# mprib/caliscope

Measured on AMD Instinct MI355X. Metric: observations/sec per LM iteration, higher is better.
Workload: dtype f64; 1 GPU; cfg4: 64 cams / 2000000 obs in total (200000 points / 2000000 obs on rank 0), extrinsics-only BA, linear loss; n_obs_total=2000000, params_per_camera=6, tolerances=ftol=xtol=gtol=1e-8 (reference defaults), sums=FP64 atomics (default)

## Files before the change

### caliscope_amd/build.py

```python

from __future__ import annotations

import os
import shutil
import subprocess
import sys
from pathlib import Path

HERE = Path(__file__).resolve().parent
CSRC = HERE / "csrc"
OUT = HERE / "libcaliscope_ba.so"
SOURCES = [CSRC / "cba_lib.hip", CSRC / "cba_solve.cpp", CSRC / "pose_lib.hip", CSRC / "scale_lib.hip", CSRC / "coverage_lib.hip", CSRC / "vertical_lib.hip", CSRC / "report_lib.hip", CSRC / "trajectory_lib.hip", CSRC / "covariance_lib.hip", CSRC / "reliability_lib.hip"]
DEPENDS = [CSRC / "cba_kernels.h", CSRC / "schur_plan.h", CSRC / "chol_schedule.h", CSRC / "chol_factor.h", CSRC / "host_plan.h", CSRC / "wg_binding.h", CSRC / "ba_math.h", CSRC / "trf_math.h", CSRC / "pnp_math.h", CSRC / "epipolar_math.h", CSRC / "intrinsic_math.h", CSRC / "frame_select_math.h", CSRC / "scale_math.h", CSRC / "coverage_math.h", CSRC / "vertical_math.h", CSRC / "report_math.h", CSRC / "trajectory_math.h", CSRC / "trajectory_refine_math.h", CSRC / "trajectory_cov_math.h", CSRC / "trajectory_smooth_math.h", CSRC / "covariance_math.h", CSRC / "covariance_constraint_math.h", CSRC / "covariance_constraint_plan.h", CSRC / "covariance_pipeline.h", CSRC / "reliability_math.h", CSRC / "reliability_constraint_math.h", CSRC / "device_call.h",
           HERE.parent / "include" / "caliscope_ba.h", HERE.parent / "include" / "caliscope_pose.h", HERE.parent / "include" / "caliscope_coverage.h", HERE.parent / "include" / "caliscope_vertical.h", HERE.parent / "include" / "caliscope_report.h", HERE.parent / "include" / "caliscope_trajectory.h", HERE.parent / "include" / "caliscope" / "uncertainty.h", HERE.parent / "include" / "caliscope" / "uncertainty_constrained.h",HERE.parent / "include" / "caliscope" / "reliability.h", HERE.parent / "include" / "caliscope" / "reliability_constrained.h",HERE.parent / "include" / "caliscope" / "trajectory_refine.h", HERE.parent / "include" / "caliscope" / "trajectory_uncertainty.h", HERE.parent / "include" / "caliscope" / "trajectory_smoother.h"]
ARCH = "gfx950"


def hipcc_path() -> str:
    for cand in (os.environ.get("HIPCC"), shutil.which("hipcc"), "/opt/rocm/bin/hipcc"):
        if cand and Path(cand).exists():
            return cand
    raise RuntimeError("hipcc not found (expected /opt/rocm/bin/hipcc)")


def needs_build() -> bool:
    if not OUT.exists():
        return True
    t = OUT.stat().st_mtime
    return any(p.stat().st_mtime > t for p in SOURCES + DEPENDS)


def source_digest() -> str:
    import hashlib

    h = hashlib.sha256()
    for path in sorted(SOURCES + DEPENDS, key=lambda q: q.name):
        h.update(path.name.encode())
        h.update(path.read_bytes())
    return h.hexdigest()


def built_digest(path: Path = OUT) -> str | None:
    import re

    m = re.search(rb"CBA_SOURCE_DIGEST=([0-9a-f]{64})", path.read_bytes())
    return m.group(1).decode() if m else None


def build(force: bool = False, verbose: bool = True) -> Path:
    if not force and not needs_build() and built_digest() == source_digest():
        return OUT
    cmd = [
        hipcc_path(), f"--offload-arch={ARCH}", "-O3", "-std=c++17", "-shared", "-fPIC", "-munsafe-fp-atomics",
        "-Wall", "-Wno-unused-function", f'-DCBA_SOURCE_DIGEST="{source_digest()}"', *map(str, SOURCES), "-o", str(OUT), "-pthread", "-lrccl",
        "-lrocprofiler-sdk-roctx",
    ]
    if verbose:
        print("[caliscope_amd.build]", " ".join(cmd), flush=True)
    subprocess.run(cmd, check=True, cwd=str(CSRC))
    return OUT


if __name__ == "__main__":
    build(force="--force" in sys.argv)
    print(OUT)
```

### caliscope_amd/csrc/ba_math.h

```cpp
#pragma once
#include <cstddef>
#include <cmath>
#include <cstdint>

#if defined(__HIPCC__)
#define CBA_HD __host__ __device__ __forceinline__
#else
#define CBA_HD inline
#endif

namespace cba {

constexpr int MODEL_PINHOLE_BC5 = 0;
constexpr int MODEL_FISHEYE4 = 1;
constexpr int CAM_CONST_STRIDE = 12;
constexpr int MAX_NC = 9;
constexpr double EPS_F64 = 2.220446049250313e-16;

CBA_HD double inv_sqrt(double x) {
#if defined(__HIP_DEVICE_COMPILE__)
  double y = __builtin_amdgcn_rsq(x);
  y = y * (1.5 - 0.5 * x * y * y);
  y = y * (1.5 - 0.5 * x * y * y);
  return y;
#else
  return 1.0 / sqrt(x);
#endif
}

enum Loss : int { LOSS_LINEAR = 0, LOSS_HUBER = 1, LOSS_SOFT_L1 = 2, LOSS_CAUCHY = 3, LOSS_ARCTAN = 4 };

struct CamTab {
  double R[9];
  double t[3];
  double Jl[9];
  double fx, fy, cx, cy;
  double d[5];
  double fx0, fy0, inv_fx0;
  double model;
  double nparams;
  double pad[13];
};
static_assert(sizeof(CamTab) == 48 * sizeof(double), "CamTab must be 48 doubles");
static_assert(offsetof(CamTab, pad) == 35 * sizeof(double), "35 doubles + pad[0] are live (CAMTAB_LIVE = 36 in cba_kernels.h)");
constexpr int CAMTAB_DOUBLES = 48;

CBA_HD void cam_prepare(const double* x_cam, const double* cconst, int model, int nparams, CamTab* o, int param_off = 0) {
  const double rx = x_cam[0], ry = x_cam[1], rz = x_cam[2];
  const double th2 = rx * rx + ry * ry + rz * rz;
  const double th = sqrt(th2);
  double ca, sa, a, b;
  if (th < 1e-4) {
    const double th4 = th2 * th2;
    a = 0.5 - th2 / 24.0 + th4 / 720.0;
    b = 1.0 / 6.0 - th2 / 120.0 + th4 / 5040.0;
    ca = 1.0 - th2 * a;
    sa = th - th2 * th * b;
  } else {
    ca = cos(th);
    sa = sin(th);
    a = (1.0 - ca) / th2;
    b = (th - sa) / (th2 * th);
  }
  const double sinc = (th < 1e-4) ? (1.0 - th2 / 6.0 + th2 * th2 / 120.0) : sa / th;
  const double xx = rx * rx, yy = ry * ry, zz = rz * rz, xy = rx * ry, xz = rx * rz, yz = ry * rz;
  o->R[0] = 1.0 + a * (xx - th2);  o->R[1] = -sinc * rz + a * xy;    o->R[2] = sinc * ry + a * xz;
  o->R[3] = sinc * rz + a * xy;    o->R[4] = 1.0 + a * (yy - th2);   o->R[5] = -sinc * rx + a * yz;
  o->R[6] = -sinc * ry + a * xz;   o->R[7] = sinc * rx + a * yz;     o->R[8] = 1.0 + a * (zz - th2);
  o->Jl[0] = 1.0 + b * (xx - th2); o->Jl[1] = -a * rz + b * xy;      o->Jl[2] = a * ry + b * xz;
  o->Jl[3] = a * rz + b * xy;      o->Jl[4] = 1.0 + b * (yy - th2);  o->Jl[5] = -a * rx + b * yz;
  o->Jl[6] = -a * ry + b * xz;     o->Jl[7] = a * rx + b * yz;       o->Jl[8] = 1.0 + b * (zz - th2);
  (void)ca;
  o->t[0] = x_cam[3]; o->t[1] = x_cam[4]; o->t[2] = x_cam[5];
  const double fx0 = cconst[0], fy0 = cconst[1];
  o->fx0 = fx0; o->fy0 = fy0; o->inv_fx0 = 1.0 / fx0;
  o->cx = cconst[2]; o->cy = cconst[3];
  const bool free_intr = nparams == 9;
  o->fx = free_intr ? x_cam[6] * fx0 : fx0;
  o->fy = free_intr ? x_cam[6] * fy0 : fy0;
  o->d[0] = free_intr ? x_cam[7] : cconst[4];
  o->d[1] = free_intr ? x_cam[8] : cconst[5];
  for (int i = 2; i < 5; ++i) o->d[i] = cconst[4 + i];
  o->model = (double)model;
  o->nparams = (double)nparams;
  o->pad[0] = (double)param_off;
  for (int i = 1; i < 13; ++i) o->pad[i] = 0.0;
}

struct Lens {
  double xd, yd;
  double dxx, dxy, dyx, dyy;
  double xr2, yr2, xr4, yr4;
};

CBA_HD void lens_pinhole(const double* d, double x, double y, Lens* L) {
  const double k1 = d[0], k2 = d[1], p1 = d[2], p2 = d[3], k3 = d[4];
  const double r2 = x * x + y * y, r4 = r2 * r2;
  const double cd = 1.0 + r2 * (k1 + r2 * (k2 + r2 * k3));
  const double dcd2 = 2.0 * (k1 + r2 * (2.0 * k2 + r2 * (3.0 * k3)));
  const double x2 = x + x, y2 = y + y;
  const double a1 = x2 * y, a2 = r2 + x2 * x, a3 = r2 + y2 * y;
  L->xd = x * cd + p1 * a1 + p2 * a2;
  L->yd = y * cd + p1 * a3 + p2 * a1;
  L->dxx = cd + x * x * dcd2 + p1 * y2 + 3.0 * p2 * x2;
  L->dxy = x * y * dcd2 + p1 * x2 + p2 * y2;
  L->dyx = L->dxy;
  L->dyy = cd + y * y * dcd2 + 3.0 * p1 * y2 + p2 * x2;
  L->xr2 = x * r2; L->yr2 = y * r2; L->xr4 = x * r4; L->yr4 = y * r4;
}

CBA_HD void lens_fisheye(const double* d, double x, double y, Lens* L) {
  const double r2 = x * x + y * y;
  const double r = sqrt(r2);
  if (r > 1e-8) {
    const double th = atan(r), t2 = th * th;
    const double poly = 1.0 + t2 * (d[0] + t2 * (d[1] + t2 * (d[2] + t2 * d[3])));
    const double dpoly = 1.0 + t2 * (3.0 * d[0] + t2 * (5.0 * d[1] + t2 * (7.0 * d[2] + t2 * 9.0 * d[3])));
    const double thd = th * poly;
    const double inv_r = 1.0 / r;
    const double cd = thd * inv_r;
    const double dcd_dr = (dpoly / (1.0 + r2) * r - thd) * inv_r * inv_r;
    const double g = dcd_dr * inv_r;
    L->xd = x * cd; L->yd = y * cd;
    L->dxx = cd + x * x * g; L->dxy = x * y * g; L->dyx = L->dxy; L->dyy = cd + y * y * g;
  } else {
    L->xd = x; L->yd = y;
    L->dxx = 1.0; L->dxy = 0.0; L->dyx = 0.0; L->dyy = 1.0;
  }
  L->xr2 = L->yr2 = L->xr4 = L->yr4 = 0.0;
}

CBA_HD void project_residual(const CamTab& c, double X, double Y, double Z, double u, double v, double* e) {
  const double Xc = c.t[0] + c.R[0] * X + c.R[1] * Y + c.R[2] * Z;
  const double Yc = c.t[1] + c.R[3] * X + c.R[4] * Y + c.R[5] * Z;
  const double Zc = c.t[2] + c.R[6] * X + c.R[7] * Y + c.R[8] * Z;
  const double iz = 1.0 / Zc;
  const double x = Xc * iz, y = Yc * iz;
  Lens L;
  if (c.model != 0.0) lens_fisheye(c.d, x, y, &L); else lens_pinhole(c.d, x, y, &L);
  e[0] = ((c.cx - u) + c.fx * L.xd) * c.inv_fx0;
  e[1] = ((c.cy - v) + c.fy * L.yd) * c.inv_fx0;
}

CBA_HD void project_full(const CamTab& c, double X, double Y, double Z, double u, double v,
                         double* e, double (*A)[MAX_NC], double (*B)[3]) {
  const double Y0 = c.R[0] * X + c.R[1] * Y + c.R[2] * Z;
  const double Y1 = c.R[3] * X + c.R[4] * Y + c.R[5] * Z;
  const double Y2 = c.R[6] * X + c.R[7] * Y + c.R[8] * Z;
  const double Zc = Y2 + c.t[2];
  const double iz = 1.0 / Zc;
  const double x = (Y0 + c.t[0]) * iz, y = (Y1 + c.t[1]) * iz;
  Lens L;
  if (c.model != 0.0) lens_fisheye(c.d, x, y, &L); else lens_pinhole(c.d, x, y, &L);
  const double s = c.inv_fx0;
  e[0] = ((c.cx - u) + c.fx * L.xd) * s;
  e[1] = ((c.cy - v) + c.fy * L.yd) * s;
  const double fxs = c.fx * s, fys = c.fy * s;
  const double g00 = fxs * L.dxx * iz, g01 = fxs * L.dxy * iz;
  const double g10 = fys * L.dyx * iz, g11 = fys * L.dyy * iz;
  const double G[2][3] = {{g00, g01, -(g00 * x + g01 * y)}, {g10, g11, -(g10 * x + g11 * y)}};
  for (int r = 0; r < 2; ++r) {
    A[r][3] = G[r][0]; A[r][4] = G[r][1]; A[r][5] = G[r][2];
    B[r][0] = G[r][0] * c.R[0] + G[r][1] * c.R[3] + G[r][2] * c.R[6];
    B[r][1] = G[r][0] * c.R[1] + G[r][1] * c.R[4] + G[r][2] * c.R[7];
    B[r][2] = G[r][0] * c.R[2] + G[r][1] * c.R[5] + G[r][2] * c.R[8];
  }
  for (int j = 0; j < 3; ++j) {
    const double m0 = c.Jl[j], m1 = c.Jl[3 + j], m2 = c.Jl[6 + j];
    const double c0 = m1 * Y2 - m2 * Y1, c1 = m2 * Y0 - m0 * Y2, c2 = m0 * Y1 - m1 * Y0;
    A[0][j] = G[0][0] * c0 + G[0][1] * c1 + G[0][2] * c2;
    A[1][j] = G[1][0] * c0 + G[1][1] * c1 + G[1][2] * c2;
  }
  if (c.nparams == 9.0) {
    A[0][6] = c.fx0 * L.xd * s; A[1][6] = c.fy0 * L.yd * s;
    A[0][7] = fxs * L.xr2;      A[1][7] = fys * L.yr2;
    A[0][8] = fxs * L.xr4;      A[1][8] = fys * L.yr4;
  }
}

template <bool RES>
CBA_HD void project_factors_impl(const CamTab& c, double X, double Y, double Z, double u, double v,
                                 double* e, double (*G)[3], double* Yr, double (*Aint)[3], double (*B)[3], double* nrm = nullptr) {
  const double Y0 = c.R[0] * X + c.R[1] * Y + c.R[2] * Z;
  const double Y1 = c.R[3] * X + c.R[4] * Y + c.R[5] * Z;
  const double Y2 = c.R[6] * X + c.R[7] * Y + c.R[8] * Z;
  Yr[0] = Y0; Yr[1] = Y1; Yr[2] = Y2;
  const double Zc = Y2 + c.t[2];
  const double iz = 1.0 / Zc;
  const double x = (Y0 + c.t[0]) * iz, y = (Y1 + c.t[1]) * iz;
  if (nrm) { nrm[0] = x; nrm[1] = y; nrm[2] = iz; }
  Lens L;
  if (c.model != 0.0) lens_fisheye(c.d, x, y, &L); else lens_pinhole(c.d, x, y, &L);
  const double s = c.inv_fx0;
  if constexpr (RES) {
    e[0] = ((c.cx - u) + c.fx * L.xd) * s;
    e[1] = ((c.cy - v) + c.fy * L.yd) * s;
  }
  const double fxs = c.fx * s, fys = c.fy * s;
  const double g00 = fxs * L.dxx * iz, g01 = fxs * L.dxy * iz;
  const double g10 = fys * L.dyx * iz, g11 = fys * L.dyy * iz;
  G[0][0] = g00; G[0][1] = g01; G[0][2] = -(g00 * x + g01 * y);
  G[1][0] = g10; G[1][1] = g11; G[1][2] = -(g10 * x + g11 * y);
  for (int r = 0; r < 2; ++r) {
    B[r][0] = G[r][0] * c.R[0] + G[r][1] * c.R[3] + G[r][2] * c.R[6];
    B[r][1] = G[r][0] * c.R[1] + G[r][1] * c.R[4] + G[r][2] * c.R[7];
    B[r][2] = G[r][0] * c.R[2] + G[r][1] * c.R[5] + G[r][2] * c.R[8];
  }
  const bool free_intr = c.nparams == 9.0;
  Aint[0][0] = free_intr ? c.fx0 * L.xd * s : 0.0; Aint[1][0] = free_intr ? c.fy0 * L.yd * s : 0.0;
  Aint[0][1] = free_intr ? fxs * L.xr2 : 0.0;      Aint[1][1] = free_intr ? fys * L.yr2 : 0.0;
  Aint[0][2] = free_intr ? fxs * L.xr4 : 0.0;      Aint[1][2] = free_intr ? fys * L.yr4 : 0.0;
}
CBA_HD void project_factors(const CamTab& c, double X, double Y, double Z, double u, double v,
                            double* e, double (*G)[3], double* Yr, double (*Aint)[3], double (*B)[3], double* nrm = nullptr) {
  project_factors_impl<true>(c, X, Y, Z, u, v, e, G, Yr, Aint, B, nrm);
}
CBA_HD void project_factors(const CamTab& c, double X, double Y, double Z, double (*G)[3], double* Yr, double (*Aint)[3], double (*B)[3],
                            double* nrm = nullptr) {
  project_factors_impl<false>(c, X, Y, Z, 0.0, 0.0, nullptr, G, Yr, Aint, B, nrm);
}

constexpr int REC6_VALUES = 10;
CBA_HD void rec6_head(const double* Yr, const double* t, double* nrm) {
  const double Zc = Yr[2] + t[2];
  const double iz = 1.0 / Zc;
  nrm[0] = (Yr[0] + t[0]) * iz; nrm[1] = (Yr[1] + t[1]) * iz; nrm[2] = iz;
}
CBA_HD void rec6_pack(const double (*G)[3], const double* Yr, const double (*Z)[3], double iz, double* rec) {
  rec[0] = Yr[0]; rec[1] = Yr[1]; rec[2] = Yr[2]; rec[3] = iz;
  for (int r = 0; r < 2; ++r)
    for (int k = 0; k < 3; ++k) rec[4 + 3 * r + k] = G[0][r] * Z[0][k] + G[1][r] * Z[1][k];
}
CBA_HD void rec6_pack(const double (*G)[3], const double* Yr, const double* t, const double (*Z)[3], double* rec) {
  double nrm[3];
  rec6_head(Yr, t, nrm);
  rec6_pack(G, Yr, Z, nrm[2], rec);
}
CBA_HD void rec6_xy(const double* rec, const double* t, double* x, double* y) {
  *x = (rec[0] + t[0]) * rec[3];
  *y = (rec[1] + t[1]) * rec[3];
}
CBA_HD void rec6_expand(const double* rec, const double* t, double* full) {
  double x, y;
  rec6_xy(rec, t, &x, &y);
  full[0] = rec[0]; full[1] = rec[1]; full[2] = rec[2];
  for (int k = 0; k < 3; ++k) {
    full[3 + k] = rec[4 + k]; full[6 + k] = rec[7 + k];
    full[9 + k] = -(x * rec[4 + k] + y * rec[7 + k]);
  }
}

CBA_HD double robust_one(int loss, double f_scale, double r, double* row_scale, double* r_scaled) {
  if (loss == LOSS_LINEAR) { *row_scale = 1.0; *r_scaled = r; return r * r; }
  const double fs2 = f_scale * f_scale;
  const double z = (r * r) / fs2;
  double rho0, rho1, rho2;
  switch (loss) {
    case LOSS_HUBER:
      if (z <= 1.0) { rho0 = z; rho1 = 1.0; rho2 = 0.0; }
      else { const double sz = sqrt(z); rho0 = 2.0 * sz - 1.0; rho1 = 1.0 / sz; rho2 = -0.5 / (z * sz); }
      break;
    case LOSS_SOFT_L1: {
      const double t = 1.0 + z, st = sqrt(t);
      rho0 = 2.0 * (st - 1.0); rho1 = 1.0 / st; rho2 = -0.5 / (t * st);
    } break;
    case LOSS_CAUCHY: {
      const double t = 1.0 + z;
      rho0 = log1p(z); rho1 = 1.0 / t; rho2 = -1.0 / (t * t);
    } break;
    default: {
      const double t = 1.0 + z * z;
      rho0 = atan(z); rho1 = 1.0 / t; rho2 = -2.0 * z / (t * t);
    } break;
  }
  double js = rho1 + 2.0 * rho2 * z;
  if (js < EPS_F64) js = EPS_F64;
  js = sqrt(js);
  *row_scale = js;
  *r_scaled = r * rho1 / js;
  return rho0 * fs2;
}

CBA_HD double robust_cost_one(int loss, double f_scale, double r) {
  if (loss == LOSS_LINEAR) return r * r;
  const double fs2 = f_scale * f_scale;
// ... 145 lines not shown
```

### caliscope_amd/csrc/cba_kernels.h

```cpp
#pragma once
#include <hip/hip_runtime.h>

#include "ba_math.h"
#include "trf_math.h"
#include "wg_binding.h"
#include "chol_schedule.h"

namespace cba {

constexpr int BLOCK = 256;
constexpr int CHUNK = 256;
constexpr int WAVE = 64;

struct VecLayout {
  int ncp;
  int ncp_pad;
  int P;
  int Ppad;
  __host__ __device__ long total() const { return (long)ncp_pad + 3L * Ppad; }
};

__device__ __forceinline__ double wave_sum(double v) {
#pragma unroll
  for (int o = WAVE / 2; o > 0; o >>= 1) v += __shfl_down(v, o, WAVE);
  return v;
}
__device__ __forceinline__ double wave_max(double v) {
#pragma unroll
  for (int o = WAVE / 2; o > 0; o >>= 1) v = fmax(v, __shfl_down(v, o, WAVE));
  return v;
}
#ifdef CBA_PROFILING
constexpr int STAMP_SLOTS = 96, STAMP_BLOCKS = 1024, STAMP_WAVES = 16, STAMP_ROW = 1 + STAMP_WAVES;
__device__ long long* g_cba_stamps = nullptr;
struct StampScope {
  long long* row;
  __device__ __forceinline__ explicit StampScope(int slot) : row(nullptr) {
    long long* base = g_cba_stamps;
    const int b = (int)(blockIdx.y * gridDim.x + blockIdx.x);
    if (base && slot < STAMP_SLOTS && b < STAMP_BLOCKS) {
      row = base + ((long)slot * STAMP_BLOCKS + b) * STAMP_ROW;
      if (threadIdx.x == 0 && threadIdx.y == 0) row[0] = wall_clock64();
    }
  }
  __device__ __forceinline__ ~StampScope() {
    const int t = (int)(threadIdx.y * blockDim.x + threadIdx.x);
    if (row && (t & (WAVE - 1)) == 0 && t / WAVE < STAMP_WAVES) row[1 + t / WAVE] = wall_clock64();
  }
};
#define CBA_STAMP(slot) StampScope cba_stamp_scope_(slot)
#else
#define CBA_STAMP(slot) ((void)0)
#endif
enum StampId { ST_TPREP = 0, ST_PAIRS, ST_REG_REDUCE, ST_FINALIZE, ST_CHOL_APPLY, ST_BACKSUB, ST_STEP_CAM, ST_BUILD, ST_REDUCE_PUB, ST_SCALE_LIN, ST_JV,
               ST_SMALL_SOLVE, ST_CHOL_STEP  };

__device__ __forceinline__ double block_sum(double v, double* sh) {
  v = wave_sum(v);
  const int lane = threadIdx.x & (WAVE - 1), w = threadIdx.x / WAVE;
  __syncthreads();
  if (lane == 0) sh[w] = v;
  __syncthreads();
  double r = 0.0;
  if (threadIdx.x == 0)
    for (int i = 0; i < BLOCK / WAVE; ++i) r += sh[i];
  return r;
}
__device__ __forceinline__ double block_max(double v, double* sh) {
  v = wave_max(v);
  const int lane = threadIdx.x & (WAVE - 1), w = threadIdx.x / WAVE;
  __syncthreads();
  if (lane == 0) sh[w] = v;
  __syncthreads();
  double r = 0.0;
  if (threadIdx.x == 0)
    for (int i = 0; i < BLOCK / WAVE; ++i) r = fmax(r, sh[i]);
  return r;
}

__device__ __forceinline__ void lds_add(double* addr, double v) { unsafeAtomicAdd(addr, v); }

constexpr int CAMTAB_LIVE = 36;
constexpr int CAMTAB_LDS = CAMTAB_LIVE + 1;
struct ObsRec { double u, v; int cam, pt; };
__device__ __forceinline__ ObsRec load_obs(const double* __restrict__ obs_u, const double* __restrict__ obs_v,
                                           const int* __restrict__ obs_cam, const int* __restrict__ obs_pt, int i) {
  ObsRec r;
  r.u = obs_u[i]; r.v = obs_v[i]; r.cam = obs_cam[i]; r.pt = obs_pt[i];
  return r;
}

__device__ __forceinline__ void stage_camtab(double* sh_tab, const double* tab, int n_cams) {
  for (int i = threadIdx.x; i < n_cams * CAMTAB_LIVE; i += BLOCK)
    sh_tab[(i / CAMTAB_LIVE) * CAMTAB_LDS + (i % CAMTAB_LIVE)] = tab[(i / CAMTAB_LIVE) * CAMTAB_DOUBLES + (i % CAMTAB_LIVE)];
}
__device__ __forceinline__ const CamTab& cam_at(const double* sh_tab, int cam) {
  return *reinterpret_cast<const CamTab*>(sh_tab + cam * CAMTAB_LDS);
}
template <bool CAMG>
__device__ __forceinline__ const CamTab& cam_of(const double* sh_tab, const double* __restrict__ tab, int cam) {
  if constexpr (CAMG) return *reinterpret_cast<const CamTab*>(tab + (long)cam * CAMTAB_DOUBLES);
  else return cam_at(sh_tab, cam);
}

__global__ void k_cam_prep(const double* __restrict__ xvec, const double* __restrict__ cam_const,
                           const int* __restrict__ cam_model, const int* __restrict__ cam_np,
                           const int* __restrict__ cam_off, int n_cams, double* __restrict__ tab) {
  const int c = blockIdx.x * blockDim.x + threadIdx.x;
  if (c >= n_cams) return;
  double xc[MAX_NC];
  const int np = cam_np[c];
  for (int i = 0; i < MAX_NC; ++i) xc[i] = (i < np) ? xvec[cam_off[c] + i] : 0.0;
  CamTab t;
  cam_prepare(xc, cam_const + c * CAM_CONST_STRIDE, cam_model[c], np, &t, cam_off[c]);
  const double* src = reinterpret_cast<const double*>(&t);
  for (int i = 0; i < CAMTAB_DOUBLES; ++i) tab[c * CAMTAB_DOUBLES + i] = src[i];
}

__global__ void __launch_bounds__(BLOCK)
k_begin(const double* __restrict__ x0, double* __restrict__ x, double* __restrict__ x_new, double* __restrict__ sinv, double* __restrict__ cam_diag,
        int* __restrict__ flags, long total, int ncp_pad, const double* __restrict__ cam_const, const int* __restrict__ cam_model,
        const int* __restrict__ cam_np, const int* __restrict__ cam_off, int n_cams, double* __restrict__ tab) {
  const long t0 = (long)blockIdx.x * blockDim.x + threadIdx.x;
  for (long i = t0; i < total; i += (long)gridDim.x * blockDim.x) {
    const double v = x0[i];
    x[i] = v;
    if (x_new) x_new[i] = v;
    sinv[i] = 1.0;
    if (i < ncp_pad) cam_diag[i] = 0.0;
    if (i < 4) flags[i] = 0;
  }
  if (t0 < n_cams) {
    const int c = (int)t0;
    double xc[MAX_NC];
    const int np = cam_np[c];
    for (int i = 0; i < MAX_NC; ++i) xc[i] = (i < np) ? x0[cam_off[c] + i] : 0.0;
    CamTab t;
    cam_prepare(xc, cam_const + c * CAM_CONST_STRIDE, cam_model[c], np, &t, cam_off[c]);
    const double* src = reinterpret_cast<const double*>(&t);
    for (int i = 0; i < CAMTAB_DOUBLES; ++i) tab[c * CAMTAB_DOUBLES + i] = src[i];
  }
}

template <bool WRITE_R, bool CAMG = false>
__global__ void __launch_bounds__(BLOCK)
k_cost(const double* __restrict__ obs_u, const double* __restrict__ obs_v, const int* __restrict__ obs_cam,
       const int* __restrict__ obs_pt, long n_obs, const double* __restrict__ xvec, VecLayout lay,
       const double* __restrict__ tab, int n_cams, int loss, double f_scale, double* __restrict__ partial,
       int* __restrict__ flags, double* __restrict__ r_out, const int* __restrict__ order) {
  extern __shared__ __attribute__((aligned(16))) double sh[];
  double* sh_tab = sh;
  double* sh_red = sh + (CAMG ? 0 : n_cams * CAMTAB_LDS);
  if (!CAMG) stage_camtab(sh_tab, tab, n_cams);
  __syncthreads();
  const double* px = xvec + lay.ncp_pad;
  double acc = 0.0;
  bool bad = false;
  struct Rec { int cam, pt; double u, v; long o; };
  const long stride = (long)gridDim.x * BLOCK, last = n_obs - 1;
  auto load_rec = [&](long i) {
    Rec r; const long k = min(i, last);
    r.cam = obs_cam[k]; r.pt = obs_pt[k]; r.u = obs_u[k]; r.v = obs_v[k]; r.o = WRITE_R ? (long)order[k] : 0;
    return r;
  };
  long i = (long)blockIdx.x * BLOCK + threadIdx.x;
  Rec rc = load_rec(i), rn = load_rec(i + stride);
  double X = px[rc.pt], Y = px[lay.Ppad + rc.pt], Z = px[2 * lay.Ppad + rc.pt];
  for (; i < n_obs; i += stride) {
    asm volatile("s_waitcnt vmcnt(0)" ::: "memory");
    asm volatile("" : "+v"(rc.cam), "+v"(rc.pt), "+v"(rc.u), "+v"(rc.v), "+v"(rc.o));
    asm volatile("" : "+v"(rn.cam), "+v"(rn.pt), "+v"(rn.u), "+v"(rn.v), "+v"(rn.o));
    asm volatile("" : "+v"(X), "+v"(Y), "+v"(Z));
    const double Xn = px[rn.pt], Yn = px[lay.Ppad + rn.pt], Zn = px[2 * lay.Ppad + rn.pt];
    const Rec rnn = load_rec(i + 2 * stride);
    __builtin_amdgcn_sched_barrier(0);
    double e[2];
    project_residual(cam_of<CAMG>(sh_tab, tab, rc.cam), X, Y, Z, rc.u, rc.v, e);
    if (!(isfinite(e[0]) && isfinite(e[1]))) bad = true;
    acc += robust_cost_one(loss, f_scale, e[0]) + robust_cost_one(loss, f_scale, e[1]);
    if (WRITE_R) {
      r_out[2 * rc.o] = e[0];
      r_out[2 * rc.o + 1] = e[1];
    }
    rc = rn; rn = rnn; X = Xn; Y = Yn; Z = Zn;
  }
  asm volatile("s_waitcnt vmcnt(0)" ::: "memory");
  if (bad) flags[0] = 1;
  const double tot = block_sum(acc, sh_red);
  if (threadIdx.x == 0) partial[blockIdx.x] = tot;
}

constexpr int REDUCE_RY = 16;
__device__ __forceinline__ void reduce_rows_block(const double* __restrict__ partial, int nrow, int width, double* __restrict__ out,
                                                  double* __restrict__ grad_out, const int* __restrict__ cam_off, const int* __restrict__ cam_np,
                                                  int stride, int tri) {
  __shared__ double sh[REDUCE_RY][64];
  const int j = blockIdx.x * 64 + threadIdx.x;
  double acc[8] = {0.0, 0.0, 0.0, 0.0, 0.0, 0.0, 0.0, 0.0};
  if (j < width) {
    int b = threadIdx.y;
    for (; b + 7 * REDUCE_RY < nrow; b += 8 * REDUCE_RY) {
#pragma unroll
      for (int q = 0; q < 8; ++q) acc[q] += partial[(long)(b + q * REDUCE_RY) * width + j];
    }
    for (; b < nrow; b += REDUCE_RY) acc[0] += partial[(long)b * width + j];
  }
  sh[threadIdx.y][threadIdx.x] = ((acc[0] + acc[1]) + (acc[2] + acc[3])) + ((acc[4] + acc[5]) + (acc[6] + acc[7]));
  __syncthreads();
  if (threadIdx.y == 0 && j < width) {
    double tot = 0.0;
#pragma unroll
    for (int y = 0; y < REDUCE_RY; ++y) tot += sh[y][threadIdx.x];
    out[j] = tot;
    if (grad_out) {
      const int c = j / stride, r = j % stride - tri;
      if (r >= 0 && r < cam_np[c]) grad_out[cam_off[c] + r] = tot;
    }
  }
}
__global__ void __launch_bounds__(64 * REDUCE_RY)
k_reduce_rows(const double* __restrict__ partial, int nrow, int width, double* __restrict__ out,
              double* __restrict__ grad_out = nullptr, const int* __restrict__ cam_off = nullptr, const int* __restrict__ cam_np = nullptr,
              int stride = 1, int tri = 0) {
  reduce_rows_block(partial, nrow, width, out, grad_out, cam_off, cam_np, stride, tri);
}
struct PubArgs {
  double* scal; int n_scal; int* flags; double* host_scal; int* host_flags; unsigned long long seq;
  const double* part_a; int rows_a, slot_a; const double* part_b; int rows_b, slot_b;
  const double* cam_src[4]; double* cam_dst; int ncp;
  int* spec_word; double ftol, xtol, cost_x;
};
__device__ __forceinline__ int pub_solve_ends(const PubArgs& pub, double ta, double tb) {
  const double cost_new = 0.5 * ta;
  const double cost = isnan(pub.cost_x) ? 0.5 * pub.scal[8] : pub.cost_x;
  if (pub.scal[42] != 0.0 || (pub.flags[0] | pub.flags[1] | pub.flags[2] | pub.flags[3]) != 0 || !isfinite(cost_new) || !isfinite(cost)) return 0;
  const double actual = cost - cost_new;
  const double ratio = trf::reduction_ratio(actual, pub.scal[45]);
  return trf::termination(actual, cost, sqrt(tb), sqrt(pub.scal[2]), ratio, pub.ftol, pub.xtol) != trf::TERMINATION_NONE ? 1 : 0;
}
__device__ __forceinline__ void publish_packet(const PubArgs& pub) {
  __shared__ double sh_w[2][REDUCE_RY];
  const int t = threadIdx.y * 64 + threadIdx.x;
  const double own = (t < pub.n_scal) ? pub.scal[t] : 0.0;
  double a = 0.0, b = 0.0;
  for (int r = t; r < pub.rows_a; r += 64 * REDUCE_RY) a += pub.part_a[r];
  for (int r = t; r < pub.rows_b; r += 64 * REDUCE_RY) b += pub.part_b[r];
  a = wave_sum(a); b = wave_sum(b);
  if (threadIdx.x == 0) { sh_w[0][threadIdx.y] = a; sh_w[1][threadIdx.y] = b; }
  __syncthreads();
  __shared__ double sh_tot[3];
  if (t == 0) {
    double ta = 0.0, tb = 0.0;
    for (int i = 0; i < REDUCE_RY; ++i) { ta += sh_w[0][i]; tb += sh_w[1][i]; }
    pub.scal[pub.slot_a] = ta; pub.scal[pub.slot_b] = tb;
    sh_tot[0] = ta; sh_tot[1] = tb;
    int ends = 0;
    if (pub.spec_word) { ends = pub_solve_ends(pub, ta, tb); *pub.spec_word = ends; }
    sh_tot[2] = (double)ends;
  }
  __syncthreads();
  if (t < pub.n_scal) pub.host_scal[t] = (t == pub.slot_a) ? sh_tot[0] : (t == pub.slot_b) ? sh_tot[1] : (t == pub.n_scal - 1) ? sh_tot[2] : own;
  if (t < 4) { pub.host_flags[t] = pub.flags[t]; pub.flags[t] = 0; }
  if (pub.cam_dst)
    for (int e = t; e < 4 * pub.ncp; e += 64 * REDUCE_RY) pub.cam_dst[e] = pub.cam_src[e / pub.ncp][e % pub.ncp];
  __threadfence_system();
  __syncthreads();
  if (t == 0) reinterpret_cast<volatile unsigned long long*>(pub.host_scal)[63] = pub.seq;
}
__global__ void __launch_bounds__(64 * REDUCE_RY)
k_reduce_rows_pub(const double* __restrict__ partial, int nrow, int width, double* __restrict__ out, double* __restrict__ grad_out,
                  const int* __restrict__ cam_off, const int* __restrict__ cam_np, int stride, int tri, PubArgs pub) {
  CBA_STAMP(ST_REDUCE_PUB);
  if (blockIdx.x + 1 < gridDim.x) { reduce_rows_block(partial, nrow, width, out, grad_out, cam_off, cam_np, stride, tri); return; }
  publish_packet(pub);
}
__global__ void k_xpack(const double* __restrict__ scal, const int* __restrict__ flags, unsigned long long mask, int with_max,
                        int rank, int world, double* __restrict__ xbuf) {
  if (threadIdx.x != 0 || blockIdx.x != 0) return;
  int n = 0;
  for (int s2 = 0; s2 < 32; ++s2)
    if ((mask >> s2) & 1ull) xbuf[n++] = scal[s2];
  for (int k = 0; k < 4; ++k) xbuf[n++] = flags[k] ? 1.0 : 0.0;
  if (with_max)
    for (int r = 0; r < world; ++r) xbuf[n++] = (r == rank) ? scal[4] : 0.0;
}
__global__ void k_xunpack(const double* __restrict__ xbuf, unsigned long long mask, int with_max, int world,
                          double* __restrict__ scal, int* __restrict__ flags) {
  if (threadIdx.x != 0 || blockIdx.x != 0) return;
  int n = 0;
  for (int s2 = 0; s2 < 32; ++s2)
    if ((mask >> s2) & 1ull) scal[s2] = xbuf[n++];
  for (int k = 0; k < 4; ++k) flags[k] = xbuf[n++] > 0.5 ? 1 : 0;
  if (with_max) {
    double m = 0.0;
    for (int r = 0; r < world; ++r) m = fmax(m, xbuf[n++]);
    scal[4] = m;
  }
}

template <bool MAX>
__global__ void __launch_bounds__(BLOCK)
k_reduce_narrow(const double* __restrict__ partial, int nrow, int width, double* __restrict__ out) {
  __shared__ double sh_red[BLOCK / WAVE];
  for (int j = 0; j < width; ++j) {
    double s = 0.0;
    for (int b = threadIdx.x; b < nrow; b += BLOCK) {
      const double v = partial[(long)b * width + j];
      s = MAX ? fmax(s, v) : s + v;
    }
    const double r = MAX ? block_max(s, sh_red) : block_sum(s, sh_red);
    if (threadIdx.x == 0) out[j] = r;
  }
}

template <int NC>
__device__ __forceinline__ double obs_linearize(const CamTab& c_lds, double X, double Y, double Z, double u, double v,
                                                int loss, double f_scale, double* e, double (*A)[MAX_NC],
                                                double (*B)[3]) {
  const CamTab c = c_lds;
  __builtin_amdgcn_sched_barrier(0);
  project_full(c, X, Y, Z, u, v, e, A, B);
  double rho = 0.0;
#pragma unroll
  for (int r = 0; r < 2; ++r) {
    double rs, er;
    rho += robust_one(loss, f_scale, e[r], &rs, &er);
    e[r] = er;
    if (loss != LOSS_LINEAR) {
#pragma unroll
      for (int k = 0; k < NC; ++k) A[r][k] *= rs;
      B[r][0] *= rs; B[r][1] *= rs; B[r][2] *= rs;
    }
  }
  return rho;
}

__device__ __forceinline__ double obs_factors(const CamTab& c_lds, double X, double Y, double Z, double u, double v, int loss, double f_scale, double* e,
                                              double (*G)[3], double* Yr, double (*Aint)[3], double (*B)[3], double* nrm = nullptr) {
  CamTab c;
  {
    const double* src = reinterpret_cast<const double*>(&c_lds);
    double* dst = reinterpret_cast<double*>(&c);
#pragma unroll
    for (int i = 0; i < 12; ++i) dst[i] = src[i];
#pragma unroll
    for (int i = 21; i < 35; ++i) dst[i] = src[i];
  }
  __builtin_amdgcn_sched_barrier(0);
  project_factors(c, X, Y, Z, u, v, e, G, Yr, Aint, B, nrm);
  if (nrm) {
#pragma unroll
    for (int k = 0; k < 3; ++k) asm("" : "+v"(nrm[k]));
  }
  double rho = 0.0;
#pragma unroll
  for (int r = 0; r < 2; ++r) {
    double rs, er;
    rho += robust_one(loss, f_scale, e[r], &rs, &er);
    e[r] = er;
    if (loss != LOSS_LINEAR) {
#pragma unroll
      for (int k = 0; k < 3; ++k) { G[r][k] *= rs; B[r][k] *= rs; Aint[r][k] *= rs; }
    }
  }
  return rho;
}
__device__ __forceinline__ void obs_factors(const CamTab& c_lds, double X, double Y, double Z, double (*G)[3], double* Yr, double (*Aint)[3], double (*B)[3],
                                            double* nrm = nullptr) {
  CamTab c;
  {
    const double* src = reinterpret_cast<const double*>(&c_lds);
    double* dst = reinterpret_cast<double*>(&c);
#pragma unroll
    for (int i = 0; i < 12; ++i) dst[i] = src[i];
    dst[21] = src[21]; dst[22] = src[22];
#pragma unroll
    for (int i = 25; i < 35; ++i) dst[i] = src[i];
  }
  __builtin_amdgcn_sched_barrier(0);
  project_factors(c, X, Y, Z, G, Yr, Aint, B, nrm);
#pragma unroll
  for (int r = 0; r < 2; ++r) {
#pragma unroll
    for (int k = 0; k < 3; ++k) { asm("" : "+v"(G[r][k])); asm("" : "+v"(B[r][k])); asm("" : "+v"(Aint[r][k])); }
  }
#pragma unroll
  for (int k = 0; k < 3; ++k) asm("" : "+v"(Yr[k]));
  if (nrm) {
#pragma unroll
    for (int k = 0; k < 3; ++k) asm("" : "+v"(nrm[k]));
  }
}

template <int NC> struct UPack {
  static constexpr int TRI = NC * (NC + 1) / 2;
  static constexpr int STRIDE = TRI + NC;
  __host__ __device__ static constexpr int idx(int r, int c) { return r * NC - r * (r - 1) / 2 + (c - r); }
};

constexpr int DET_ROUND = 9;
constexpr int DET_LD = CHUNK + 1;
struct DetPlan {
  const unsigned char* perm;
  const unsigned short* cstart;
};
template <int M>
__device__ __forceinline__ void det_round(const double* val, double* sh_cv, const int* sh_perm, const int* sh_cs, int n_cams, double* acc) {
#pragma unroll
  for (int q = 0; q < DET_ROUND; ++q) sh_cv[q * DET_LD + threadIdx.x] = val[q];
  __syncthreads();
#pragma unroll
  for (int m = 0; m < M; ++m) {
    const int task = (int)threadIdx.x + BLOCK * m;
    if (task < n_cams * DET_ROUND) {
      const int c = task / DET_ROUND, q = task % DET_ROUND;
      double s = 0.0;
      for (int j = sh_cs[c]; j < sh_cs[c + 1]; ++j) s += sh_cv[q * DET_LD + sh_perm[j]];
      acc[m] += s;
    }
  }
  __syncthreads();
}

template <int NC>
__device__ __forceinline__ double cam_block_value(int v, const double (*A)[MAX_NC], const double* e, int np) {
  using UP = UPack<NC>;
  int idx = 0;
#pragma unroll
  for (int r = 0; r < NC; ++r)
#pragma unroll
    for (int c = r; c < NC; ++c, ++idx)
      if (idx == v) return (r < np && c < np) ? A[0][r] * A[0][c] + A[1][r] * A[1][c] : 0.0;
#pragma unroll
  for (int r = 0; r < NC; ++r)
    if (UP::TRI + r == v) return (r < np) ? A[0][r] * e[0] + A[1][r] * e[1] : 0.0;
  return 0.0;
}

template <int NC, int DETM = 0, bool CAMG = false>
__global__ void __launch_bounds__(BLOCK)
k_build(const double* __restrict__ obs_u, const double* __restrict__ obs_v, const int* __restrict__ obs_cam,
        const int* __restrict__ obs_pt, const int* __restrict__ pt_start, const int* __restrict__ chunk_start,
        const int* __restrict__ chunk_pts, int n_chunks, const double* __restrict__ xvec, VecLayout lay, const double* __restrict__ tab, int n_cams,
        int loss, double f_scale, double* __restrict__ Vblk, double* __restrict__ gvec,
        double* __restrict__ partialU, double* __restrict__ partial_cost, int* __restrict__ flags, const double* __restrict__ skip,
        DetPlan det = DetPlan{nullptr, nullptr}) {
  using UP = UPack<NC>;
  constexpr bool DET = DETM > 0;
  if (skip && *skip != 0.0) return;
  extern __shared__ __attribute__((aligned(16))) double sh[];
  double* sh_tab = sh;
  double* sh_U = sh_tab + (CAMG ? 0 : n_cams * CAMTAB_LDS);
  auto cam_of = [&](int cam) -> const CamTab& {
    return CAMG ? *reinterpret_cast<const CamTab*>(tab + (long)cam * CAMTAB_DOUBLES) : cam_at(sh_tab, cam);
  };
  double* sh_pt = sh_U + (DET ? DET_ROUND * DET_LD : n_cams * UP::STRIDE);
  double* sh_red = sh_pt + 9 * CHUNK;
  int* sh_perm = reinterpret_cast<int*>(sh_red + 8);
  int* sh_cs = sh_perm + CHUNK;
  constexpr int DROUNDS = (UP::STRIDE + DET_ROUND - 1) / DET_ROUND;
  constexpr int DM = DET ? DETM : 1;
  double dacc[DROUNDS][DM];
#pragma unroll
  for (int r = 0; r < DROUNDS; ++r)
#pragma unroll
    for (int m = 0; m < DM; ++m) dacc[r][m] = 0.0;
  if (!CAMG) stage_camtab(sh_tab, tab, n_cams);
  if (!DET)
    for (int i = threadIdx.x; i < n_cams * UP::STRIDE; i += BLOCK) sh_U[i] = 0.0;
  __syncthreads();
  const double* px = xvec + lay.ncp_pad;
  double* gp = gvec + lay.ncp_pad;
  double cost = 0.0;
  bool bad = false;
  const int last_obs = max(chunk_start[n_chunks] - 1, 0);
  int ch = blockIdx.x;
  int o0 = 0, o1 = 0;
  ObsRec cur = {0.0, 0.0, 0, 0};
  if (ch < n_chunks) {
    o0 = chunk_start[ch]; o1 = chunk_start[ch + 1];
    cur = load_obs(obs_u, obs_v, obs_cam, obs_pt, min(o0 + (int)threadIdx.x, last_obs));
  }
  while (ch < n_chunks) {
    const int nxt = ch + gridDim.x, nc = min(nxt, n_chunks - 1);
    const int no0 = chunk_start[nc], no1 = chunk_start[nc + 1];
    const ObsRec nx = load_obs(obs_u, obs_v, obs_cam, obs_pt, min(no0 + (int)threadIdx.x, last_obs));
    const int cp0 = chunk_pts[2 * ch], npts = chunk_pts[2 * ch + 1];
    const int pp = min(cp0 + (int)threadIdx.x, lay.P - 1);
    const int pa = pt_start[pp] - o0, pb = pt_start[pp + 1] - o0;
    const int i = o0 + threadIdx.x;
    double pv[9];
#pragma unroll
    for (int q = 0; q < 9; ++q) pv[q] = 0.0;
    double e[2] = {0.0, 0.0}, A[2][MAX_NC];
    int np_det = 0;
    if (DET) {
#pragma unroll
      for (int k = 0; k < MAX_NC; ++k) { A[0][k] = 0.0; A[1][k] = 0.0; }
      sh_perm[threadIdx.x] = det.perm[(long)ch * CHUNK + threadIdx.x];
      for (int q = threadIdx.x; q <= n_cams; q += BLOCK) sh_cs[q] = det.cstart[(long)ch * (n_cams + 1) + q];
    }
    if (i < o1) {
      const int cam = cur.cam, pt = cur.pt;
      double B[2][3];
      cost += obs_linearize<NC>(cam_of(cam), px[pt], px[lay.Ppad + pt], px[2 * lay.Ppad + pt], cur.u, cur.v, loss,
                                f_scale, e, A, B);
      if (!isfinite(e[0] + e[1])) bad = true;
      pv[0] = B[0][0] * B[0][0] + B[1][0] * B[1][0];
      pv[1] = B[0][0] * B[0][1] + B[1][0] * B[1][1];
      pv[2] = B[0][0] * B[0][2] + B[1][0] * B[1][2];
      pv[3] = B[0][1] * B[0][1] + B[1][1] * B[1][1];
      pv[4] = B[0][1] * B[0][2] + B[1][1] * B[1][2];
      pv[5] = B[0][2] * B[0][2] + B[1][2] * B[1][2];
      pv[6] = B[0][0] * e[0] + B[1][0] * e[1];
      pv[7] = B[0][1] * e[0] + B[1][1] * e[1];
      pv[8] = B[0][2] * e[0] + B[1][2] * e[1];
      const int np = (int)cam_of(cam).nparams;
      np_det = np;
      if (!DET) {
        double* Uc = sh_U + cam * UP::STRIDE;
#pragma unroll
        for (int r = 0; r < NC; ++r) {
          if (r < np) {
#pragma unroll
            for (int c = r; c < NC; ++c)
              if (c < np) lds_add(&Uc[UP::idx(r, c)], A[0][r] * A[0][c] + A[1][r] * A[1][c]);
            lds_add(&Uc[UP::TRI + r], A[0][r] * e[0] + A[1][r] * e[1]);
          }
        }
      }
    }
#pragma unroll
    for (int q = 0; q < 9; ++q) sh_pt[q * CHUNK + threadIdx.x] = pv[q];
    __syncthreads();
    auto reduce_point = [&](int p, int a, int b) {
      double acc[9];
#pragma unroll
      for (int q = 0; q < 9; ++q) acc[q] = 0.0;
      for (int j = a; j < b; ++j) {
#pragma unroll
        for (int q = 0; q < 9; ++q) acc[q] += sh_pt[q * CHUNK + j];
      }
#pragma unroll
      for (int q = 0; q < 6; ++q) Vblk[(long)q * lay.Ppad + p] = acc[q];
      gp[p] = acc[6];
      gp[lay.Ppad + p] = acc[7];
      gp[2 * lay.Ppad + p] = acc[8];
    };
    if (npts < 0 && threadIdx.x < 9) {
      double acc = 0.0;
      for (int j = 0; j < o1 - o0; ++j) acc += sh_pt[threadIdx.x * CHUNK + j];
      if (threadIdx.x < 6) unsafeAtomicAdd(&Vblk[(long)threadIdx.x * lay.Ppad + cp0], acc);
      else unsafeAtomicAdd(&gp[(long)(threadIdx.x - 6) * lay.Ppad + cp0], acc);
    }
    if ((int)threadIdx.x < npts && pb > pa) reduce_point(pp, pa, pb);
    for (int lp = threadIdx.x + BLOCK; lp < npts; lp += BLOCK) {
      const int p = cp0 + lp;
      const int a = pt_start[p] - o0, b = pt_start[p + 1] - o0;
      if (b > a) reduce_point(p, a, b);
    }
    __syncthreads();
    if (DET) {
#pragma unroll
      for (int rd = 0; rd < DROUNDS; ++rd) {
        double val[DET_ROUND];
#pragma unroll
        for (int q = 0; q < DET_ROUND; ++q) val[q] = cam_block_value<NC>(rd * DET_ROUND + q, A, e, np_det);
        det_round<DM>(val, sh_U, sh_perm, sh_cs, n_cams, dacc[rd]);
      }
    }
    cur = nx; o0 = no0; o1 = no1; ch = nxt;
  }
  double* dst = partialU + (long)blockIdx.x * n_cams * UP::STRIDE;
  if (DET) {
#pragma unroll
    for (int rd = 0; rd < DROUNDS; ++rd)
#pragma unroll
      for (int m = 0; m < DM; ++m) {
        const int task = (int)threadIdx.x + BLOCK * m;
        const int c = task / DET_ROUND, v = rd * DET_ROUND + task % DET_ROUND;
        if (task < n_cams * DET_ROUND && v < UP::STRIDE) dst[c * UP::STRIDE + v] = dacc[rd][m];
      }
  } else {
    for (int i = threadIdx.x; i < n_cams * UP::STRIDE; i += BLOCK) dst[i] = sh_U[i];
  }
  const double tot = block_sum(cost, sh_red);
  if (threadIdx.x == 0) partial_cost[blockIdx.x] = tot;
  if (bad) flags[0] = 1;
}

constexpr int CS_MAX_PTS = 512;
struct CsPlan {
  const double* u;
  const double* v;
  const int* cam;
  const int* ptl;
  const int* obs_start;
  const int* pt_first;
  const int* pt_count;
  int n_sc;
  int pmax;
};
struct TrialSrc {
  const double *x, *g, *sinv, *s;
  const double* ab;
  double* x_new;
  double* step_partial;
};
template <int NC, bool CAMG = false, bool UGLOB = false, bool TRIAL = false>
__global__ void __launch_bounds__(BLOCK)
k_build_cs(CsPlan cs, const double* __restrict__ xvec, VecLayout lay, const double* __restrict__ tab, int n_cams, int loss, double f_scale,
           double* __restrict__ Vblk, double* __restrict__ gvec, double* __restrict__ partialU, double* __restrict__ partial_cost,
           int* __restrict__ flags, const double* __restrict__ skip, TrialSrc trial = TrialSrc{}) {
  CBA_STAMP(ST_BUILD);
  using UP = UPack<NC>;
  static_assert(!UGLOB || CAMG, "a camera count beyond the LDS copy of the blocks is beyond the LDS copy of the table as well");
  if (skip && *skip != 0.0) return;
  extern __shared__ __attribute__((aligned(16))) double sh[];
  double* sh_tab = sh;
  double* sh_U = sh_tab + (CAMG ? 0 : n_cams * CAMTAB_LDS);
  const int PM = cs.pmax;
  double* sh_vg = sh_U + (UGLOB ? 0 : n_cams * UP::STRIDE);
  double* sh_x = sh_vg + 9 * PM;
  double* sh_red = sh_x + 3 * PM;
  if (!CAMG) stage_camtab(sh_tab, tab, n_cams);
  if (!UGLOB)
    for (int i = threadIdx.x; i < n_cams * UP::STRIDE; i += BLOCK) sh_U[i] = 0.0;
  const double* px = xvec + lay.ncp_pad;
  double* gp = gvec + lay.ncp_pad;
  double cost = 0.0, step_sq = 0.0;
  const double t_alpha = TRIAL ? trial.ab[0] : 0.0, t_beta = TRIAL ? trial.ab[1] : 0.0;
  bool bad = false;
  for (int s = blockIdx.x; s < cs.n_sc; s += gridDim.x) {
    const int o0 = cs.obs_start[s], o1 = cs.obs_start[s + 1], p0 = cs.pt_first[s], npts = cs.pt_count[s];
    __syncthreads();
    for (int i = threadIdx.x; i < 9 * PM; i += BLOCK) sh_vg[i] = 0.0;
    if (TRIAL) {
      for (int i = threadIdx.x; i < npts; i += BLOCK) {
#pragma unroll
        for (int k = 0; k < 3; ++k) {
          const long e = (long)lay.ncp_pad + (long)k * lay.Ppad + p0 + i;
          const double si = trial.sinv[e];
          const double st = t_alpha * trial.g[e] / (si * si) + t_beta * trial.s[e];
          const double xn = trial.x[e] + st;
          trial.x_new[e] = xn;
          sh_x[k * PM + i] = xn;
          step_sq = fma(st, st, step_sq);
        }
      }
    } else {
      for (int i = threadIdx.x; i < npts; i += BLOCK) {
        sh_x[i] = px[p0 + i]; sh_x[PM + i] = px[lay.Ppad + p0 + i]; sh_x[2 * PM + i] = px[2 * lay.Ppad + p0 + i];
      }
    }
    __syncthreads();
    const int R = (o1 - o0 + BLOCK - 1) / BLOCK;
    const int j0 = o0 + (int)threadIdx.x * R, j1 = min(j0 + R, o1);
    double acc[UP::STRIDE];
#pragma unroll
    for (int q = 0; q < UP::STRIDE; ++q) acc[q] = 0.0;
    int cur_cam = -1, cur_np = 0;
    auto flush = [&]() {
      if (cur_cam < 0) return;
      double* Uc = (UGLOB ? partialU : sh_U) + (long)cur_cam * UP::STRIDE;
#pragma unroll
      for (int r = 0; r < NC; ++r) {
        if (r < cur_np) {
#pragma unroll
          for (int c = r; c < NC; ++c)
            if (c < cur_np) { if (UGLOB) atomicAdd(&Uc[UP::idx(r, c)], acc[UP::idx(r, c)]); else lds_add(&Uc[UP::idx(r, c)], acc[UP::idx(r, c)]); }
          if (UGLOB) atomicAdd(&Uc[UP::TRI + r], acc[UP::TRI + r]); else lds_add(&Uc[UP::TRI + r], acc[UP::TRI + r]);
        }
      }
#pragma unroll
      for (int q = 0; q < UP::STRIDE; ++q) acc[q] = 0.0;
    };
    const int jl = max(o1 - 1, 0);
    int n_cam = cs.cam[min(j0, jl)], n_pl = cs.ptl[min(j0, jl)];
    double n_u = cs.u[min(j0, jl)], n_v = cs.v[min(j0, jl)];
    for (int j = j0; j < j1; ++j) {
      asm volatile("s_waitcnt vmcnt(0)" ::: "memory");
      asm volatile("" : "+v"(n_cam), "+v"(n_pl), "+v"(n_u), "+v"(n_v));
      const int cam = n_cam, pl = n_pl;
      const double u = n_u, v = n_v;
      n_cam = cs.cam[min(j + 1, jl)]; n_pl = cs.ptl[min(j + 1, jl)]; n_u = cs.u[min(j + 1, jl)]; n_v = cs.v[min(j + 1, jl)];
      __builtin_amdgcn_sched_barrier(0);
      if (cam != cur_cam) { flush(); cur_cam = cam; cur_np = (int)cam_of<CAMG>(sh_tab, tab, cam).nparams; }
      double e[2], A[2][MAX_NC], B[2][3];
      {
        double G[2][3], Yr[3], Aint[2][3];
        const CamTab& ctc = cam_of<CAMG>(sh_tab, tab, cam);
        cost += obs_factors(ctc, sh_x[pl], sh_x[PM + pl], sh_x[2 * PM + pl], u, v, loss, f_scale, e, G, Yr, Aint, B);
#pragma unroll
        for (int r = 0; r < 2; ++r) {
          const double p0 = Yr[1] * G[r][2] - Yr[2] * G[r][1], p1 = Yr[2] * G[r][0] - Yr[0] * G[r][2], p2 = Yr[0] * G[r][1] - Yr[1] * G[r][0];
          if constexpr (UGLOB) {
            A[r][0] = ctc.Jl[0] * p0 + ctc.Jl[3] * p1 + ctc.Jl[6] * p2;
            A[r][1] = ctc.Jl[1] * p0 + ctc.Jl[4] * p1 + ctc.Jl[7] * p2;
            A[r][2] = ctc.Jl[2] * p0 + ctc.Jl[5] * p1 + ctc.Jl[8] * p2;
          } else {
            A[r][0] = p0; A[r][1] = p1; A[r][2] = p2;
          }
          A[r][3] = G[r][0]; A[r][4] = G[r][1]; A[r][5] = G[r][2];
          A[r][6] = Aint[r][0]; A[r][7] = Aint[r][1]; A[r][8] = Aint[r][2];
        }
      }
      if (!isfinite(e[0] + e[1])) bad = true;
#pragma unroll
      for (int r = 0; r < NC; ++r) {
#pragma unroll
        for (int c = r; c < NC; ++c) acc[UP::idx(r, c)] = fma(A[1][r], A[1][c], fma(A[0][r], A[0][c], acc[UP::idx(r, c)]));
        acc[UP::TRI + r] = fma(A[1][r], e[1], fma(A[0][r], e[0], acc[UP::TRI + r]));
      }
      lds_add(&sh_vg[0 * PM + pl], B[0][0] * B[0][0] + B[1][0] * B[1][0]);
      lds_add(&sh_vg[1 * PM + pl], B[0][0] * B[0][1] + B[1][0] * B[1][1]);
      lds_add(&sh_vg[2 * PM + pl], B[0][0] * B[0][2] + B[1][0] * B[1][2]);
      lds_add(&sh_vg[3 * PM + pl], B[0][1] * B[0][1] + B[1][1] * B[1][1]);
      lds_add(&sh_vg[4 * PM + pl], B[0][1] * B[0][2] + B[1][1] * B[1][2]);
      lds_add(&sh_vg[5 * PM + pl], B[0][2] * B[0][2] + B[1][2] * B[1][2]);
      lds_add(&sh_vg[6 * PM + pl], B[0][0] * e[0] + B[1][0] * e[1]);
      lds_add(&sh_vg[7 * PM + pl], B[0][1] * e[0] + B[1][1] * e[1]);
      lds_add(&sh_vg[8 * PM + pl], B[0][2] * e[0] + B[1][2] * e[1]);
    }
    flush();
    __syncthreads();
    for (int i = threadIdx.x; i < npts; i += BLOCK) {
#pragma unroll
      for (int q = 0; q < 6; ++q) Vblk[(long)q * lay.Ppad + p0 + i] = sh_vg[q * PM + i];
      gp[p0 + i] = sh_vg[6 * PM + i];
      gp[lay.Ppad + p0 + i] = sh_vg[7 * PM + i];
      gp[2 * lay.Ppad + p0 + i] = sh_vg[8 * PM + i];
    }
  }
  __syncthreads();
  if (!UGLOB) {
    for (int c = threadIdx.x; c < n_cams; c += BLOCK) {
      const double* Jl = tab + (long)c * CAMTAB_DOUBLES + 12;
      double* Uc = sh_U + (long)c * UP::STRIDE;
      double M[3][3], T[3][3];
#pragma unroll
      for (int r = 0; r < 3; ++r)
#pragma unroll
        for (int q = 0; q < 3; ++q) M[r][q] = Uc[UP::idx(min(r, q), max(r, q))];
#pragma unroll
      for (int r = 0; r < 3; ++r)
#pragma unroll
        for (int q = 0; q < 3; ++q) T[r][q] = Jl[r] * M[0][q] + Jl[3 + r] * M[1][q] + Jl[6 + r] * M[2][q];
#pragma unroll
      for (int r = 0; r < 3; ++r)
#pragma unroll
        for (int q = r; q < 3; ++q) Uc[UP::idx(r, q)] = T[r][0] * Jl[q] + T[r][1] * Jl[3 + q] + T[r][2] * Jl[6 + q];
#pragma unroll
      for (int q = 3; q <= NC; ++q) {
        double* v0 = (q < NC) ? &Uc[UP::idx(0, q)] : &Uc[UP::TRI + 0];
        double* v1 = (q < NC) ? &Uc[UP::idx(1, q)] : &Uc[UP::TRI + 1];
        double* v2 = (q < NC) ? &Uc[UP::idx(2, q)] : &Uc[UP::TRI + 2];
        const double a0 = *v0, a1 = *v1, a2 = *v2;
        *v0 = Jl[0] * a0 + Jl[3] * a1 + Jl[6] * a2;
        *v1 = Jl[1] * a0 + Jl[4] * a1 + Jl[7] * a2;
        *v2 = Jl[2] * a0 + Jl[5] * a1 + Jl[8] * a2;
      }
    }
    __syncthreads();
    double* dst = partialU + (long)blockIdx.x * n_cams * UP::STRIDE;
    for (int i = threadIdx.x; i < n_cams * UP::STRIDE; i += BLOCK) dst[i] = sh_U[i];
  }
  const double tot = block_sum(cost, sh_red);
  if (threadIdx.x == 0) partial_cost[blockIdx.x] = tot;
  if (TRIAL) {
    const double st = block_sum(step_sq, sh_red);
    if (threadIdx.x == 0) trial.step_partial[blockIdx.x] = st;
  }
  if (bad) flags[0] = 1;
}

__global__ void __launch_bounds__(256)
k_gather_uv(const double* __restrict__ uv_raw, const int* __restrict__ order, long n, double* __restrict__ u, double* __restrict__ v) {
  for (long i = (long)blockIdx.x * 256 + threadIdx.x; i < n; i += (long)gridDim.x * 256) {
    const double2 w = reinterpret_cast<const double2*>(uv_raw)[order[i]];
    u[i] = w.x; v[i] = w.y;
  }
}
__global__ void __launch_bounds__(256)
k_cs_fill(const int* __restrict__ perm, const int* __restrict__ sc_obs, const int* __restrict__ sc_p0, const double* __restrict__ u,
          const double* __restrict__ v, const int* __restrict__ cam, const int* __restrict__ pt, double* __restrict__ cu, double* __restrict__ cv,
          int* __restrict__ ccam, int* __restrict__ cptl) {
  const int s = blockIdx.x, o0 = sc_obs[s], o1 = sc_obs[s + 1], p0 = sc_p0[s];
  for (int j = o0 + threadIdx.x; j < o1; j += 256) {
    const int i = perm[j];
    cu[j] = u[i]; cv[j] = v[i]; ccam[j] = cam[i]; cptl[j] = pt[i] - p0;
  }
}

template <int NC>
__global__ void k_unpack_camera_grad(const double* __restrict__ Upacked, const int* __restrict__ cam_off,
                                     const int* __restrict__ cam_np, int n_cams, double* __restrict__ gvec) {
  using UP = UPack<NC>;
  const int t = blockIdx.x * blockDim.x + threadIdx.x;
  const int c = t / NC, r = t % NC;
  if (c >= n_cams || r >= cam_np[c]) return;
  gvec[cam_off[c] + r] = Upacked[c * UP::STRIDE + UP::TRI + r];
}

template <int NC>
__global__ void k_scale_update(const double* __restrict__ Upacked, const double* __restrict__ Vblk,
                               const int* __restrict__ param_cam, const int* __restrict__ param_loc, VecLayout lay,
                               int first, double* __restrict__ sinv, const double* __restrict__ cdiag) {
  using UP = UPack<NC>;
  const long total = lay.total();
  for (long i = (long)blockIdx.x * blockDim.x + threadIdx.x; i < total; i += (long)gridDim.x * blockDim.x) {
    double v;
    if (i < lay.ncp_pad) {
      if (i >= lay.ncp) continue;
      const int r = param_loc[i];
      v = Upacked[param_cam[i] * UP::STRIDE + UP::idx(r, r)];
    } else {
      const long k = (i - lay.ncp_pad) / lay.Ppad, p = (i - lay.ncp_pad) % lay.Ppad;
      if (p >= lay.P) continue;
      const int q = (k == 0) ? 0 : (k == 1 ? 3 : 5);
      v = Vblk[(long)q * lay.Ppad + p];
      if (cdiag) v += cdiag[k * lay.Ppad + p];
    }
    v = sqrt(v);
    if (first) { if (v == 0.0) v = 1.0; }
    else v = fmax(v, sinv[i]);
    sinv[i] = v;
  }
}

__global__ void k_cam_rescale(const double* __restrict__ state, const double* __restrict__ mult, const double* __restrict__ diag_h,
                              int ncp, double* __restrict__ sinv, double* __restrict__ cam_diag) {
  const int i = blockIdx.x * blockDim.x + threadIdx.x;
  if (i >= ncp) return;
  const double si = state[i] * mult[i];
  sinv[i] = si;
  cam_diag[i] = diag_h[i] * si * si;
}

__global__ void __launch_bounds__(BLOCK)
k_lin_scalars(const double* __restrict__ x, const double* __restrict__ g, const double* __restrict__ sinv,
              long total, int cam_end, int count_cams, int max_from, double* __restrict__ v1, double* __restrict__ partial,
              double* __restrict__ partial_max) {
  __shared__ double sh_red[BLOCK / WAVE];
  double s0 = 0, s1 = 0, s2 = 0, m = 0;
  for (long i = (long)blockIdx.x * BLOCK + threadIdx.x; i < total; i += (long)gridDim.x * BLOCK) {
    const double gi = g[i], si = sinv[i], xi = x[i];
    const double gh = gi / si;
    v1[i] = gh / si;
    if (i >= max_from) m = fmax(m, fabs(gi));
    if (i < cam_end && !count_cams) continue;
    s0 += gh * gh;
    s1 += (xi * si) * (xi * si);
    s2 += xi * xi;
  }
  double r;
  r = block_sum(s0, sh_red); if (threadIdx.x == 0) partial[blockIdx.x * 4 + 0] = r;
  r = block_sum(s1, sh_red); if (threadIdx.x == 0) partial[blockIdx.x * 4 + 1] = r;
  r = block_sum(s2, sh_red); if (threadIdx.x == 0) partial[blockIdx.x * 4 + 2] = r;
  if (threadIdx.x == 0) partial[blockIdx.x * 4 + 3] = 0.0;
  r = block_max(m, sh_red); if (threadIdx.x == 0) partial_max[blockIdx.x] = r;
}

__global__ void k_combine(const double* __restrict__ g, const double* __restrict__ sinv, const double* __restrict__ s,
                          double a, double b, long total, const double* __restrict__ over, int n_over, double* __restrict__ out) {
  for (long i = (long)blockIdx.x * blockDim.x + threadIdx.x; i < total; i += (long)gridDim.x * blockDim.x) {
    const double si = sinv[i];
    out[i] = (i < n_over) ? over[i] : a * g[i] / (si * si) + b * s[i];
  }
}

constexpr int MAIL_GNORM = 60, MAIL_GNORM_SEQ = 61;
struct SpecSkip {
  const int* word;
  const double* max_rows;
  int n_rows;
  double* mail; unsigned long long seq;
};
__device__ __forceinline__ void publish_gnorm(const SpecSkip& sk) {
  __shared__ double sh_gn[BLOCK / WAVE];
  double m = 0.0;
  for (int b = threadIdx.x; b < sk.n_rows; b += BLOCK) m = fmax(m, sk.max_rows[b]);
  m = block_max(m, sh_gn);
  if (threadIdx.x == 0) {
    sk.mail[MAIL_GNORM] = m;
    __threadfence_system();
    reinterpret_cast<volatile unsigned long long*>(sk.mail)[MAIL_GNORM_SEQ] = sk.seq;
  }
}
__global__ void __launch_bounds__(BLOCK) k_gnorm_pub(SpecSkip sk) { publish_gnorm(sk); }

template <int NC, int NV, bool CAMG = false, bool LIN = false>
__global__ void __launch_bounds__(BLOCK)
k_jv(const double* __restrict__ obs_u, const double* __restrict__ obs_v, const int* __restrict__ obs_cam,
     const int* __restrict__ obs_pt, long n_obs, const double* __restrict__ xvec, VecLayout lay,
     const double* __restrict__ tab, const int* __restrict__ cam_off, int n_cams, int loss, double f_scale,
     const double* __restrict__ v1, const double* __restrict__ v2, double* __restrict__ partial, SpecSkip skip = SpecSkip{}) {
  CBA_STAMP(ST_JV);
  if (skip.word && *skip.word) {
    if (blockIdx.x == 0) publish_gnorm(skip);
    return;
  }
  extern __shared__ __attribute__((aligned(16))) double sh[];
  double* sh_tab = sh;
  double* sh_v = sh_tab + (CAMG ? 0 : n_cams * CAMTAB_LDS);
  double* sh_red = sh_v + NV * lay.ncp_pad;
  if (!CAMG) stage_camtab(sh_tab, tab, n_cams);
  for (int i = threadIdx.x; i < lay.ncp_pad; i += BLOCK) {
    sh_v[i] = v1[i];
    if (NV == 2) sh_v[lay.ncp_pad + i] = v2[i];
  }
  __syncthreads();
  for (int c = threadIdx.x; c < n_cams; c += BLOCK) {
    const double* row = tab + (long)c * CAMTAB_DOUBLES;
    const int off = (int)row[35];
#pragma unroll
    for (int q = 0; q < NV; ++q) {
      double* vq = sh_v + q * lay.ncp_pad + off;
      const double r0 = vq[0], r1 = vq[1], r2 = vq[2];
      vq[0] = row[12] * r0 + row[13] * r1 + row[14] * r2;
      vq[1] = row[15] * r0 + row[16] * r1 + row[17] * r2;
      vq[2] = row[18] * r0 + row[19] * r1 + row[20] * r2;
    }
  }
  __syncthreads();
  const double* px = xvec + lay.ncp_pad;
  const double* p1 = v1 + lay.ncp_pad;
  const double* p2 = (NV == 2) ? v2 + lay.ncp_pad : nullptr;
  double s11 = 0, s12 = 0, s22 = 0;
  struct Rec { int cam, pt; double u, v; };
  struct Gat { double X, Y, Z, a, b, c, d, e, f; };
  constexpr int LOADS = (LIN ? 2 : 4) + (NV == 2 ? 9 : 6);
  const long stride = (long)gridDim.x * BLOCK, last = n_obs - 1;
  auto load_rec = [&](long i) {
    Rec r; const long k = min(i, last); r.cam = obs_cam[k]; r.pt = obs_pt[k];
    if constexpr (LIN) { r.u = r.v = 0.0; } else { r.u = obs_u[k]; r.v = obs_v[k]; }
    return r;
  };
  auto load_gat = [&](int pt) {
    Gat g;
    g.X = px[pt]; g.Y = px[lay.Ppad + pt]; g.Z = px[2 * lay.Ppad + pt];
    g.a = p1[pt]; g.b = p1[lay.Ppad + pt]; g.c = p1[2 * lay.Ppad + pt];
    if (NV == 2) { g.d = p2[pt]; g.e = p2[lay.Ppad + pt]; g.f = p2[2 * lay.Ppad + pt]; } else { g.d = g.e = g.f = 0.0; }
    return g;
  };
  auto launder_rec = [](Rec& r) {
    asm volatile("" : "+v"(r.cam), "+v"(r.pt));
    if constexpr (!LIN) asm volatile("" : "+v"(r.u), "+v"(r.v));
  };
  auto launder_gat = [](Gat& g) {
    asm volatile("" : "+v"(g.X), "+v"(g.Y), "+v"(g.Z), "+v"(g.a), "+v"(g.b), "+v"(g.c));
    if (NV == 2) asm volatile("" : "+v"(g.d), "+v"(g.e), "+v"(g.f));
  };
  long i = (long)blockIdx.x * BLOCK + threadIdx.x;
  Rec rc = load_rec(i), r1 = load_rec(i + stride), r2 = load_rec(i + 2 * stride), r3 = load_rec(i + 3 * stride);
  Gat gc = load_gat(rc.pt), g1 = load_gat(r1.pt);
  asm volatile("s_waitcnt vmcnt(0)" ::: "memory");
  launder_rec(rc); launder_rec(r1); launder_rec(r2); launder_rec(r3); launder_gat(gc); launder_gat(g1);
  for (; i < n_obs; i += stride) {
    asm volatile("s_waitcnt vmcnt(%0)" ::"n"(LOADS) : "memory");
    launder_gat(gc); launder_rec(r2);
    const Gat g2 = load_gat(r2.pt);
    const Rec r4 = load_rec(i + 4 * stride);
    __builtin_amdgcn_sched_barrier(0);
    const int cam = rc.cam;
    double e[2], G[2][3], Yr[3], Aint[2][3], B[2][3];
    const CamTab& ctj = cam_of<CAMG>(sh_tab, tab, cam);
    if constexpr (LIN) obs_factors(ctj, gc.X, gc.Y, gc.Z, G, Yr, Aint, B);
    else obs_factors(ctj, gc.X, gc.Y, gc.Z, rc.u, rc.v, loss, f_scale, e, G, Yr, Aint, B);
    const double* vc = sh_v + (int)ctj.pad[0];
    auto jv = [&](const double* q, double px0, double px1, double px2, double* o0, double* o1) {
      const double m0 = fma(q[1], Yr[2], fma(-q[2], Yr[1], q[3]));
      const double m1 = fma(q[2], Yr[0], fma(-q[0], Yr[2], q[4]));
      const double m2 = fma(q[0], Yr[1], fma(-q[1], Yr[0], q[5]));
      double a0 = B[0][0] * px0 + B[0][1] * px1 + B[0][2] * px2, a1 = B[1][0] * px0 + B[1][1] * px1 + B[1][2] * px2;
      a0 = fma(G[0][2], m2, fma(G[0][1], m1, fma(G[0][0], m0, a0)));
      a1 = fma(G[1][2], m2, fma(G[1][1], m1, fma(G[1][0], m0, a1)));
      if (NC == 9 && ctj.nparams == 9.0) {
        a0 = fma(Aint[0][2], q[8], fma(Aint[0][1], q[7], fma(Aint[0][0], q[6], a0)));
        a1 = fma(Aint[1][2], q[8], fma(Aint[1][1], q[7], fma(Aint[1][0], q[6], a1)));
      }
      *o0 = a0; *o1 = a1;
    };
    double a0, a1;
    jv(vc, gc.a, gc.b, gc.c, &a0, &a1);
    s11 += a0 * a0 + a1 * a1;
    if (NV == 2) {
      double b0, b1;
      jv(vc + lay.ncp_pad, gc.d, gc.e, gc.f, &b0, &b1);
      s12 += a0 * b0 + a1 * b1;
      s22 += b0 * b0 + b1 * b1;
    }
    rc = r1; r1 = r2; r2 = r3; r3 = r4; gc = g1; g1 = g2;
  }
  asm volatile("s_waitcnt vmcnt(0)" ::: "memory");
  double r;
  r = block_sum(s11, sh_red); if (threadIdx.x == 0) partial[blockIdx.x * 4 + 0] = r;
  r = block_sum(s12, sh_red); if (threadIdx.x == 0) partial[blockIdx.x * 4 + 1] = r;
  r = block_sum(s22, sh_red); if (threadIdx.x == 0) partial[blockIdx.x * 4 + 2] = r;
  if (threadIdx.x == 0) partial[blockIdx.x * 4 + 3] = 0.0;
}

struct TilePlan {
  const int* chunk_start;
  const int* wg_first;
  const int* wg_end;
  const int* wg_tile;
  const int* wg_stride;
  const int* tile_a;
  const int* tile_b;
  const int* group_cam_begin;
  const int* group_par_begin;
  int g;
  int tile_elems;
  const int* obs;
  int rep;
  const unsigned* codes;
  const int* code_start;
  const unsigned* nit;
  int prio_shift;
};

template <int NC> struct SchurRec {
  static constexpr int NVAL = (NC == 9) ? 21 : 10;
  static constexpr int NPH = (NVAL + 1) / 2;
  static constexpr int LST = (NPH & 1) ? NPH : NPH + 1;
  static constexpr int REC = 2 * LST;
  static constexpr int HREC = 2 * NPH;
  static constexpr int STAGE = (HREC / 2) | 1;
  static constexpr int STAGE_WAVES = (NC == 9) ? 2 : 4;
};
static_assert(SchurRec<6>::REC == 10 && SchurRec<6>::LST == 5 && SchurRec<6>::HREC == 10 && SchurRec<6>::STAGE == 5 && SchurRec<9>::REC == 22 &&
                  SchurRec<9>::LST == 11,
              "record sizes");

template <int NC>
__device__ __forceinline__ void expand_record(const double* __restrict__ rec, const double* __restrict__ cam_row, double* __restrict__ T) {
  const double* Jl = cam_row + 12;
  double full[12];
  if constexpr (NC == 6) rec6_expand(rec, cam_row + 9 , full);
  const double Y0 = (NC == 6) ? full[0] : rec[0], Y1 = (NC == 6) ? full[1] : rec[1], Y2 = (NC == 6) ? full[2] : rec[2];
  const double* Q = (NC == 6) ? full + 3 : rec + 3;
#pragma unroll
  for (int m = 0; m < 3; ++m) {
    const double q0 = Q[m], q1 = Q[3 + m], q2 = Q[6 + m];
    const double c0 = Y1 * q2 - Y2 * q1, c1 = Y2 * q0 - Y0 * q2, c2 = Y0 * q1 - Y1 * q0;
#pragma unroll
    for (int r = 0; r < 3; ++r) T[3 * r + m] = Jl[r] * c0 + Jl[3 + r] * c1 + Jl[6 + r] * c2;
    T[9 + m] = q0; T[12 + m] = q1; T[15 + m] = q2;
  }
  if (NC == 9) {
#pragma unroll
    for (int k = 0; k < 9; ++k) T[18 + k] = rec[12 + k];
  }
}

struct LinFin {
  const double* partial_lin;
  const double* partial_max;
  const double* partial_jv;
  int rows_lin, rows_jv;
  double radius;
  double* scal;
  double* fz;
};
__device__ __forceinline__ double lin_finish_block(const LinFin& lf, double (*sh_red)[BLOCK / WAVE], double* sh_out) {
  double v[10];
#pragma unroll
  for (int q = 0; q < 10; ++q) v[q] = 0.0;
  for (int b = threadIdx.x; b < lf.rows_lin; b += BLOCK) {
#pragma unroll
    for (int j = 0; j < 4; ++j) v[j] += lf.partial_lin[(long)b * 4 + j];
    v[4] = fmax(v[4], lf.partial_max[b]);
  }
  for (int b = threadIdx.x; b < lf.rows_jv; b += BLOCK) {
#pragma unroll
    for (int j = 0; j < 4; ++j) v[5 + j] += lf.partial_jv[(long)b * 4 + j];
  }
  const int lane = threadIdx.x & (WAVE - 1), w = threadIdx.x / WAVE;
#pragma unroll
  for (int q = 0; q < 9; ++q) {
    const double r = (q == 4) ? wave_max(v[q]) : wave_sum(v[q]);
    if (lane == 0) sh_red[q][w] = r;
  }
  __syncthreads();
  if (threadIdx.x == 0) {
    double tot[9];
#pragma unroll
    for (int q = 0; q < 9; ++q) {
      double r = 0.0;
      for (int i = 0; i < BLOCK / WAVE; ++i) r = (q == 4) ? fmax(r, sh_red[q][i]) : r + sh_red[q][i];
      tot[q] = r;
    }
    const double gh_sq = tot[0], jg_sq = tot[5] + tot[3], xs = sqrt(tot[1]);
    const double radius = lf.radius > 0.0 ? lf.radius : (xs > 0.0 ? xs : 1.0);
    const double lam = trf::damping(jg_sq, gh_sq, radius);
    sh_out[0] = lam;
    if (blockIdx.x == 0) {
#pragma unroll
      for (int q = 0; q < 9; ++q) lf.scal[q < 5 ? q : 12 + (q - 5)] = tot[q];
      lf.fz[0] = lam; lf.fz[1] = radius;
      lf.scal[40] = lam; lf.scal[41] = radius;
    }
  }
  __syncthreads();
  return sh_out[0];
}

template <int NC, int DETM = 0, bool CAMG = false, bool LINF = false, bool LIN = false>
__global__ void __launch_bounds__(BLOCK, DETM == 0 ? 2 : 1)
k_tprep(const double* __restrict__ obs_u, const double* __restrict__ obs_v, const int* __restrict__ obs_cam,
        const int* __restrict__ obs_pt, const int* __restrict__ chunk_start, int n_chunks,
        const double* __restrict__ xvec, VecLayout lay, const double* __restrict__ tab, const int* __restrict__ cam_off,
        int n_cams, int loss, double f_scale, double lam, const double* __restrict__ lam_dev, const double* __restrict__ Vblk,
        const double* __restrict__ gvec, const double* __restrict__ sinv, double* __restrict__ Trec,
        double* __restrict__ partial_b, int* __restrict__ flags, DetPlan det = DetPlan{nullptr, nullptr}, LinFin lf = LinFin{}) {
  CBA_STAMP(ST_TPREP);
  constexpr int REC = SchurRec<NC>::HREC, NP = REC / 2, SP = SchurRec<NC>::STAGE, SW = SchurRec<NC>::STAGE_WAVES;
  static_assert((BLOCK / WAVE) % SW == 0, "stage turns");
  constexpr bool DET = DETM > 0;
  static_assert(!(DET && CAMG), "the fixed-order sums keep the camera table in LDS");
  if (LINF) {
    __shared__ double sh_lf_red[10][BLOCK / WAVE];
    __shared__ double sh_lf_out[2];
    lam = lin_finish_block(lf, sh_lf_red, sh_lf_out);
  } else if (lam_dev) lam = *lam_dev;
  extern __shared__ __attribute__((aligned(16))) double sh[];
  double2* sh_stage = reinterpret_cast<double2*>(sh);
  double* sh_tab = sh + (size_t)SW * WAVE * SP * 2;
  double* sh_b = sh_tab + (CAMG ? 0 : n_cams * CAMTAB_LDS);
  int* sh_perm = reinterpret_cast<int*>(sh_b + DET_ROUND * DET_LD);
  int* sh_cs = sh_perm + CHUNK;
  constexpr int DM = DET ? DETM : 1;
  double dacc[DM];
#pragma unroll
  for (int m = 0; m < DM; ++m) dacc[m] = 0.0;
  stage_camtab(sh_tab, tab, n_cams);
  if (!DET)
    for (int i = threadIdx.x; i < lay.ncp_pad; i += BLOCK) sh_b[i] = 0.0;
  __syncthreads();
  const double* px = xvec + lay.ncp_pad;
  const double* gp = gvec + lay.ncp_pad;
  const double* dp = sinv + lay.ncp_pad;
  const int wv = threadIdx.x / WAVE, lane = threadIdx.x % WAVE;
  double2* stage = sh_stage + (wv % SW) * WAVE * SP;
  bool fail = false;
  const int last_obs = max(chunk_start[n_chunks] - 1, 0);
  constexpr bool PIPE = DETM == 0, FULL = true;
  struct PtOps { double X, Y, Z, V[6], d[3], g[3]; };
  auto load_rest = [&](PtOps& q, int pt) {
#pragma unroll
    for (int k = 0; k < 6; ++k) q.V[k] = Vblk[(long)k * lay.Ppad + pt];
#pragma unroll
    for (int k = 0; k < 3; ++k) { q.d[k] = dp[(long)k * lay.Ppad + pt]; q.g[k] = gp[(long)k * lay.Ppad + pt]; }
  };
  auto load_xyz = [&](PtOps& q, int pt) { q.X = px[pt]; q.Y = px[lay.Ppad + pt]; q.Z = px[2 * lay.Ppad + pt]; };
  auto load_ops = [&](int pt) {
    PtOps q;
    load_xyz(q, pt);
    if constexpr (FULL) load_rest(q, pt);
    return q;
  };
  auto load_rec = [&](int i) {
    if constexpr (LIN) return ObsRec{0.0, 0.0, obs_cam[i], obs_pt[i]};
    else return load_obs(obs_u, obs_v, obs_cam, obs_pt, i);
  };
  auto launder_obs = [](ObsRec& r) {
    if constexpr (!LIN) asm volatile("" : "+v"(r.u), "+v"(r.v));
    asm volatile("" : "+v"(r.cam), "+v"(r.pt));
  };
  auto launder_ops = [](PtOps& q) {
    asm volatile("" : "+v"(q.X), "+v"(q.Y), "+v"(q.Z));
    if constexpr (FULL) {
#pragma unroll
      for (int k = 0; k < 6; ++k) asm volatile("" : "+v"(q.V[k]));
#pragma unroll
      for (int k = 0; k < 3; ++k) asm volatile("" : "+v"(q.d[k]), "+v"(q.g[k]));
    }
  };
  const int stride = (int)gridDim.x, last_chunk = n_chunks - 1;
  int ch = blockIdx.x;
  int o0 = 0, o1 = 0, no0 = 0, no1 = 0;
  ObsRec cur = {0.0, 0.0, 0, 0}, nx = cur;
  PtOps ops;
  if (ch < n_chunks) {
    o0 = chunk_start[ch]; o1 = chunk_start[ch + 1];
    const int c1 = min(ch + stride, last_chunk);
    no0 = chunk_start[c1]; no1 = chunk_start[c1 + 1];
    cur = load_rec(min(o0 + (int)threadIdx.x, last_obs));
    if constexpr (PIPE) {
      if constexpr (FULL) nx = load_rec(min(no0 + (int)threadIdx.x, last_obs));
      else nx.pt = obs_pt[min(no0 + (int)threadIdx.x, last_obs)];
      ops = load_ops(cur.pt);
      asm volatile("s_waitcnt vmcnt(0)" ::: "memory");
      launder_obs(cur); launder_obs(nx); launder_ops(ops);
    }
  }
  while (ch < n_chunks) {
    const int nxt = ch + stride, c2 = min(ch + 2 * stride, last_chunk);
    const int nno0 = chunk_start[c2], nno1 = chunk_start[c2 + 1];
    PtOps ops_n;
    if constexpr (!PIPE) { load_xyz(ops, cur.pt); load_rest(ops, cur.pt); }
    else {
      if constexpr (!FULL) load_rest(ops, cur.pt);
      ops_n = load_ops(nx.pt);
    }
    ObsRec nn = {0.0, 0.0, 0, 0};
    if constexpr (PIPE && !FULL) {
      const int k1 = min(no0 + (int)threadIdx.x, last_obs);
      if constexpr (!LIN) { nx.u = obs_u[k1]; nx.v = obs_v[k1]; }
      nx.cam = obs_cam[k1];
      nn.pt = obs_pt[min(nno0 + (int)threadIdx.x, last_obs)];
    } else {
      nn = load_rec(min((PIPE ? nno0 : no0) + (int)threadIdx.x, last_obs));
    }
    if constexpr (PIPE) __builtin_amdgcn_sched_barrier(0);
    const int i = o0 + threadIdx.x;
    double rec[REC];
#pragma unroll
    for (int k = 0; k < REC; ++k) rec[k] = 0.0;
    double bval[DET_ROUND];
#pragma unroll
    for (int q = 0; q < DET_ROUND; ++q) bval[q] = 0.0;
    if (DET) {
      sh_perm[threadIdx.x] = det.perm[(long)ch * CHUNK + threadIdx.x];
      for (int q = threadIdx.x; q <= n_cams; q += BLOCK) sh_cs[q] = det.cstart[(long)ch * (n_cams + 1) + q];
    }
    if (i < o1) {
      const int cam = cur.cam;
      const CamTab& ct = cam_of<CAMG>(sh_tab, tab, cam);
      const double X = ops.X, Yw = ops.Y, Zw = ops.Z;
      double e[2], G[2][3], Yr[3], Aint[2][3], B[2][3], Z[2][3], nrm[3];
      if constexpr (LIN) obs_factors(ct, X, Yw, Zw, G, Yr, Aint, B, NC == 6 ? nrm : nullptr);
      else obs_factors(ct, X, Yw, Zw, cur.u, cur.v, loss, f_scale, e, G, Yr, Aint, B, NC == 6 ? nrm : nullptr);
      const int np = (int)ct.nparams;
      double Vd[6], L[6];
#pragma unroll
      for (int q = 0; q < 6; ++q) Vd[q] = ops.V[q];
      const double d0 = ops.d[0], d1 = ops.d[1], d2 = ops.d[2];
      Vd[0] += lam * d0 * d0; Vd[3] += lam * d1 * d1; Vd[5] += lam * d2 * d2;
      if (!chol3(Vd, L)) {
        fail = true;
        L[0] = L[2] = L[5] = 1.0; L[1] = L[3] = L[4] = 0.0;
      }
      chol3_fwd(L, B[0], Z[0]);
      chol3_fwd(L, B[1], Z[1]);
      const double gpt[3] = {ops.g[0], ops.g[1], ops.g[2]};
      double y[3];
      chol3_fwd(L, gpt, y);
      double* bc = sh_b + (int)ct.pad[0];
      rec[0] = Yr[0]; rec[1] = Yr[1]; rec[2] = Yr[2];
      double qy[3];
      if constexpr (NC == 6) {
        rec[3] = nrm[2];
#pragma unroll
        for (int r = 3; r < 5; ++r) {
          const double a0 = G[0][r - 3], a1 = G[1][r - 3];
          double t[3];
#pragma unroll
          for (int k = 0; k < 3; ++k) t[k] = a0 * Z[0][k] + a1 * Z[1][k];
          qy[r - 3] = t[0] * y[0] + t[1] * y[1] + t[2] * y[2];
          rec[3 * r - 5] = t[0]; rec[3 * r - 4] = t[1]; rec[3 * r - 3] = t[2];
        }
        qy[2] = -fma(nrm[0], qy[0], nrm[1] * qy[1]);
#pragma unroll
        for (int r = 3; r < 6; ++r) {
          if (DET) bval[r] = qy[r - 3];
          else lds_add(&bc[r], qy[r - 3]);
        }
      } else {
#pragma unroll
        for (int r = 3; r < NC; ++r) {
          const bool live = r < np;
          const double a0 = (r < 6) ? G[0][r - 3] : Aint[0][(r - 6) % 3], a1 = (r < 6) ? G[1][r - 3] : Aint[1][(r - 6) % 3];
          double t[3];
#pragma unroll
          for (int k = 0; k < 3; ++k) t[k] = live ? a0 * Z[0][k] + a1 * Z[1][k] : 0.0;
          const double ty = t[0] * y[0] + t[1] * y[1] + t[2] * y[2];
          if (r < 6) qy[r - 3] = ty;
          if (DET) bval[r] = live ? ty : 0.0;
          else if (live) lds_add(&bc[r], ty);
          rec[3 * r - 6] = t[0]; rec[3 * r - 5] = t[1]; rec[3 * r - 4] = t[2];
        }
      }
      {
        const double c0 = Yr[1] * qy[2] - Yr[2] * qy[1], c1 = Yr[2] * qy[0] - Yr[0] * qy[2], c2 = Yr[0] * qy[1] - Yr[1] * qy[0];
        if (DET) {
#pragma unroll
          for (int r = 0; r < 3; ++r) bval[r] = ct.Jl[r] * c0 + ct.Jl[3 + r] * c1 + ct.Jl[6 + r] * c2;
        } else {
          lds_add(&bc[0], c0); lds_add(&bc[1], c1); lds_add(&bc[2], c2);
        }
      }
    }
    if constexpr (PIPE) {
      asm volatile("s_waitcnt vmcnt(0)" ::: "memory");
      if constexpr (FULL) launder_obs(nn); else { launder_obs(nx); asm volatile("" : "+v"(nn.pt)); }
      launder_ops(ops_n);
    }
    const int w0 = o0 + wv * WAVE;
    const int n_pieces = max(0, min(WAVE, o1 - w0)) * NP;
    double2* dst = reinterpret_cast<double2*>(Trec + (long)w0 * REC);
#pragma unroll
    for (int turn = 0; turn < (BLOCK / WAVE) / SW; ++turn) {
      if (wv / SW == turn) {
#pragma unroll
        for (int k = 0; k < NP; ++k) stage[lane * SP + k] = make_double2(rec[2 * k], rec[2 * k + 1]);
        __builtin_amdgcn_fence(__ATOMIC_RELEASE, "wavefront");
        __builtin_amdgcn_wave_barrier();
        __builtin_amdgcn_fence(__ATOMIC_ACQUIRE, "wavefront");
#pragma unroll
        for (int k = 0; k < NP; ++k) {
          const int e = k * WAVE + lane;
          const double2 v = stage[(e / NP) * SP + e % NP];
          if (e < n_pieces) dst[e] = v;
        }
        __builtin_amdgcn_fence(__ATOMIC_RELEASE, "wavefront");
        __builtin_amdgcn_wave_barrier();
        __builtin_amdgcn_fence(__ATOMIC_ACQUIRE, "wavefront");
      }
      if (SW < BLOCK / WAVE) __syncthreads();
    }
    if (DET) {
      __syncthreads();
      det_round<DM>(bval, sh_b, sh_perm, sh_cs, n_cams, dacc);
    }
    if constexpr (PIPE && FULL) { cur = nx; nx = nn; ops = ops_n; }
    else if constexpr (PIPE) { cur = nx; nx.pt = nn.pt; ops.X = ops_n.X; ops.Y = ops_n.Y; ops.Z = ops_n.Z; }
    else { cur = nn; }
    o0 = no0; o1 = no1; no0 = nno0; no1 = nno1; ch = nxt;
  }
  if (fail) flags[1] = 1;
  __syncthreads();
  double* brow = partial_b + (long)blockIdx.x * lay.ncp_pad;
  if (DET) {
    for (int i = lay.ncp + threadIdx.x; i < lay.ncp_pad; i += BLOCK) brow[i] = 0.0;
#pragma unroll
    for (int m = 0; m < DM; ++m) {
      const int task = (int)threadIdx.x + BLOCK * m;
      const int c = task / DET_ROUND, q = task % DET_ROUND;
      if (task < n_cams * DET_ROUND && q < (int)cam_at(sh_tab, c).nparams) brow[cam_off[c] + q] = dacc[m];
    }
  } else {
    for (int c = threadIdx.x; c < n_cams; c += BLOCK) {
      const double* row = tab + (long)c * CAMTAB_DOUBLES;
      double* b3 = sh_b + (int)row[35];
      const double c0 = b3[0], c1 = b3[1], c2 = b3[2];
#pragma unroll
      for (int r = 0; r < 3; ++r) b3[r] = row[12 + r] * c0 + row[15 + r] * c1 + row[18 + r] * c2;
    }
    __syncthreads();
    for (int i = threadIdx.x; i < lay.ncp_pad; i += BLOCK) brow[i] = sh_b[i];
  }
}

__device__ __forceinline__ void pair9_corner(double (&acc)[6][6], const double2* __restrict__ Ri, const double2* __restrict__ Rj) {
  double D[3][3], Yi[3], Yj[3];
  {
    const double2 i0 = Ri[0], i1 = Ri[1], i2 = Ri[2], i3 = Ri[3], i4 = Ri[4], i5 = Ri[5];
    const double2 j0 = Rj[0], j1 = Rj[1], j2 = Rj[2], j3 = Rj[3], j4 = Rj[4], j5 = Rj[5];
    Yi[0] = i0.x; Yi[1] = i0.y; Yi[2] = i1.x; Yj[0] = j0.x; Yj[1] = j0.y; Yj[2] = j1.x;
    const double Qi[9] = {i1.y, i2.x, i2.y, i3.x, i3.y, i4.x, i4.y, i5.x, i5.y};
    const double Qj[9] = {j1.y, j2.x, j2.y, j3.x, j3.y, j4.x, j4.y, j5.x, j5.y};
#pragma unroll
    for (int a = 0; a < 3; ++a)
#pragma unroll
      for (int b = 0; b < 3; ++b) D[a][b] = fma(Qi[3 * a + 2], Qj[3 * b + 2], fma(Qi[3 * a + 1], Qj[3 * b + 1], Qi[3 * a] * Qj[3 * b]));
  }
  auto put = [&](int c, double m0, double m1, double m2) {
    acc[0][c] = fma(Yi[1], m2, fma(-Yi[2], m1, acc[0][c]));
    acc[1][c] = fma(Yi[2], m0, fma(-Yi[0], m2, acc[1][c]));
    acc[2][c] = fma(Yi[0], m1, fma(-Yi[1], m0, acc[2][c]));
    acc[3][c] += m0; acc[4][c] += m1; acc[5][c] += m2;
  };
#pragma unroll
  for (int b = 0; b < 3; ++b) put(3 + b, D[0][b], D[1][b], D[2][b]);
  put(0, fma(Yj[1], D[0][2], -(Yj[2] * D[0][1])), fma(Yj[1], D[1][2], -(Yj[2] * D[1][1])), fma(Yj[1], D[2][2], -(Yj[2] * D[2][1])));
  put(1, fma(Yj[2], D[0][0], -(Yj[0] * D[0][2])), fma(Yj[2], D[1][0], -(Yj[0] * D[1][2])), fma(Yj[2], D[2][0], -(Yj[0] * D[2][2])));
  put(2, fma(Yj[0], D[0][1], -(Yj[1] * D[0][0])), fma(Yj[0], D[1][1], -(Yj[1] * D[1][0])), fma(Yj[0], D[2][1], -(Yj[1] * D[2][0])));
}
__device__ __forceinline__ void pair9_cols(double* __restrict__ acc , const double2* __restrict__ Ri, const double2* __restrict__ Rj) {
  const double2 i0 = Ri[0], i1 = Ri[1], i2 = Ri[2], i3 = Ri[3], i4 = Ri[4], i5 = Ri[5], i6 = Ri[6], i7 = Ri[7], i8 = Ri[8], i9 = Ri[9], i10 = Ri[10];
  const double2 j6 = Rj[6], j7 = Rj[7], j8 = Rj[8], j9 = Rj[9], j10 = Rj[10];
  const double Yi[3] = {i0.x, i0.y, i1.x};
  const double Qi[9] = {i1.y, i2.x, i2.y, i3.x, i3.y, i4.x, i4.y, i5.x, i5.y};
  const double Ii[9] = {i6.x, i6.y, i7.x, i7.y, i8.x, i8.y, i9.x, i9.y, i10.x};
  const double Ij[9] = {j6.x, j6.y, j7.x, j7.y, j8.x, j8.y, j9.x, j9.y, j10.x};
#pragma unroll
  for (int b = 0; b < 3; ++b) {
    const double e0 = fma(Qi[2], Ij[3 * b + 2], fma(Qi[1], Ij[3 * b + 1], Qi[0] * Ij[3 * b]));
    const double e1 = fma(Qi[5], Ij[3 * b + 2], fma(Qi[4], Ij[3 * b + 1], Qi[3] * Ij[3 * b]));
    const double e2 = fma(Qi[8], Ij[3 * b + 2], fma(Qi[7], Ij[3 * b + 1], Qi[6] * Ij[3 * b]));
    acc[0 * 3 + b] = fma(Yi[1], e2, fma(-Yi[2], e1, acc[0 * 3 + b]));
    acc[1 * 3 + b] = fma(Yi[2], e0, fma(-Yi[0], e2, acc[1 * 3 + b]));
    acc[2 * 3 + b] = fma(Yi[0], e1, fma(-Yi[1], e0, acc[2 * 3 + b]));
    acc[3 * 3 + b] += e0; acc[4 * 3 + b] += e1; acc[5 * 3 + b] += e2;
#pragma unroll
    for (int a = 0; a < 3; ++a)
      acc[(6 + a) * 3 + b] = fma(Ii[3 * a + 2], Ij[3 * b + 2], fma(Ii[3 * a + 1], Ij[3 * b + 1], fma(Ii[3 * a], Ij[3 * b], acc[(6 + a) * 3 + b])));
  }
}
__device__ __forceinline__ void pair9_rows(double* __restrict__ acc , const double2* __restrict__ Ri, const double2* __restrict__ Rj) {
  const double2 i6 = Ri[6], i7 = Ri[7], i8 = Ri[8], i9 = Ri[9], i10 = Ri[10];
  const double2 j0 = Rj[0], j1 = Rj[1], j2 = Rj[2], j3 = Rj[3], j4 = Rj[4], j5 = Rj[5];
  const double Ii[9] = {i6.x, i6.y, i7.x, i7.y, i8.x, i8.y, i9.x, i9.y, i10.x};
  const double Yj[3] = {j0.x, j0.y, j1.x};
  const double Qj[9] = {j1.y, j2.x, j2.y, j3.x, j3.y, j4.x, j4.y, j5.x, j5.y};
#pragma unroll
  for (int a = 0; a < 3; ++a) {
    const double f0 = fma(Ii[3 * a + 2], Qj[2], fma(Ii[3 * a + 1], Qj[1], Ii[3 * a] * Qj[0]));
    const double f1 = fma(Ii[3 * a + 2], Qj[5], fma(Ii[3 * a + 1], Qj[4], Ii[3 * a] * Qj[3]));
    const double f2 = fma(Ii[3 * a + 2], Qj[8], fma(Ii[3 * a + 1], Qj[7], Ii[3 * a] * Qj[6]));
    acc[a * 6 + 3] += f0; acc[a * 6 + 4] += f1; acc[a * 6 + 5] += f2;
    acc[a * 6 + 0] = fma(Yj[1], f2, fma(-Yj[2], f1, acc[a * 6 + 0]));
    acc[a * 6 + 1] = fma(Yj[2], f0, fma(-Yj[0], f2, acc[a * 6 + 1]));
    acc[a * 6 + 2] = fma(Yj[0], f1, fma(-Yj[1], f0, acc[a * 6 + 2]));
  }
}

template <int NC> struct Reg3Cfg {
  static constexpr int REC = SchurRec<NC>::REC, LST = SchurRec<NC>::LST;
  static constexpr int SPLIT = (NC == 9) ? 3 : 1;
  static constexpr int CODE_THREADS = BLOCK, CODE_WAVES = BLOCK / WAVE;
  static constexpr int REG_BLOCK = BLOCK * SPLIT, NWAVES = REG_BLOCK / WAVE;
  static constexpr int GROUP = 16;
  static constexpr int NCD = (NC == 6) ? 8 : 4;
  static constexpr int PAIR_CAP = 0;
  static constexpr int SCHUNK = (NC == 9) ? 384 : 320;
  static constexpr int EPW = SCHUNK / NWAVES;
  static constexpr int NLD = (EPW * LST + WAVE - 1) / WAVE;
  static constexpr int WAVE_PIECES = NLD * WAVE;
  static constexpr int ZERO_PIECE = NWAVES * WAVE_PIECES;
  static constexpr int BUF_PIECES = ZERO_PIECE + LST + 1;
  static constexpr int NBUF = 2;
  static constexpr int SET_PIECES = NBUF * BUF_PIECES;
  static constexpr bool LANE_TABLE = (NC == 9);
  static constexpr int TABLE_PIECES = LANE_TABLE ? (NLD * WAVE * 4 + 15) / 16 : 0;
  static constexpr size_t LDS_BYTES = (size_t)(SET_PIECES + TABLE_PIECES) * 16;
  static constexpr int LAUNCH_THREADS = REG_BLOCK;
  static_assert(SCHUNK % NWAVES == 0 && EPW % 16 == 0 && EPW <= 2 * WAVE && (LST & 1) == 1, "staging layout");
  static_assert(ZERO_PIECE + LST < 65536, "piece addresses are 16 bit");
  static_assert(CODE_WAVES % 4 == 0, "iteration counts: four waves per word");
};

static_assert(Reg3Cfg<6>::EPW == 80 && Reg3Cfg<6>::LST == 5 && Reg3Cfg<6>::NLD == 7 && Reg3Cfg<6>::WAVE_PIECES == 448 && Reg3Cfg<6>::SCHUNK == 320 &&
                  Reg3Cfg<6>::ZERO_PIECE == 1792,
              "six-parameter pair kernel layout");

__device__ __forceinline__ void pair6(double (&acc)[6][6], const double2* __restrict__ Ri, const double2* __restrict__ Rj, double ti0, double ti1, double tj0,
                                      double tj1) {
  typedef double piece_t __attribute__((ext_vector_type(2)));
  const piece_t* Pi = reinterpret_cast<const piece_t*>(Ri);
  const piece_t* Pj = reinterpret_cast<const piece_t*>(Rj);
  const piece_t i0 = Pi[0], i1 = Pi[1], i2 = Pi[2], i3 = Pi[3], i4 = Pi[4];
  const piece_t j0 = Pj[0], j1 = Pj[1], j2 = Pj[2], j3 = Pj[3], j4 = Pj[4];
  const double Yi[3] = {i0.x, i0.y, i1.x}, Yj[3] = {j0.x, j0.y, j1.x};
  const double xi = (Yi[0] + ti0) * i1.y, yi = (Yi[1] + ti1) * i1.y, xj = (Yj[0] + tj0) * j1.y, yj = (Yj[1] + tj1) * j1.y;
  const double Qi[6] = {i2.x, i2.y, i3.x, i3.y, i4.x, i4.y};
  const double Qj[6] = {j2.x, j2.y, j3.x, j3.y, j4.x, j4.y};
  double M[3][6];
#pragma unroll
  for (int a = 0; a < 2; ++a) {
#pragma unroll
    for (int b2 = 0; b2 < 2; ++b2)
      M[a][3 + b2] = fma(Qi[3 * a + 2], Qj[3 * b2 + 2], fma(Qi[3 * a + 1], Qj[3 * b2 + 1], Qi[3 * a] * Qj[3 * b2]));
    M[a][5] = -fma(xj, M[a][3], yj * M[a][4]);
  }
#pragma unroll
  for (int b2 = 0; b2 < 3; ++b2) M[2][3 + b2] = -fma(xi, M[0][3 + b2], yi * M[1][3 + b2]);
#pragma unroll
  for (int a = 0; a < 3; ++a) {
    M[a][0] = fma(Yj[1], M[a][5], -(Yj[2] * M[a][4]));
    M[a][1] = fma(Yj[2], M[a][3], -(Yj[0] * M[a][5]));
    M[a][2] = fma(Yj[0], M[a][4], -(Yj[1] * M[a][3]));
  }
#pragma unroll
  for (int c = 0; c < 6; ++c) {
    acc[0][c] = fma(Yi[1], M[2][c], fma(-Yi[2], M[1][c], acc[0][c]));
    acc[1][c] = fma(Yi[2], M[0][c], fma(-Yi[0], M[2][c], acc[1][c]));
    acc[2][c] = fma(Yi[0], M[1][c], fma(-Yi[1], M[0][c], acc[2][c]));
    acc[3][c] += M[0][c]; acc[4][c] += M[1][c]; acc[5][c] += M[2][c];
  }
}

template <int NC, int RH>
__device__ __forceinline__ void unprime_rows(double (&acc)[RH][NC], int r0, const double* __restrict__ Ji, const double* __restrict__ Jj) {
  if (r0 == 0) {
#pragma unroll
    for (int c = 0; c < NC; ++c) {
      const double b0 = acc[0][c], b1 = acc[1][c], b2 = acc[2][c];
#pragma unroll
      for (int r = 0; r < 3; ++r) acc[r][c] = Ji[r] * b0 + Ji[3 + r] * b1 + Ji[6 + r] * b2;
    }
  }
#pragma unroll
  for (int r = 0; r < RH; ++r) {
    const double a0 = acc[r][0], a1 = acc[r][1], a2 = acc[r][2];
#pragma unroll
    for (int c = 0; c < 3; ++c) acc[r][c] = a0 * Jj[c] + a1 * Jj[3 + c] + a2 * Jj[6 + c];
  }
}

template <int NC, int SPLIT, bool CLK = false>
__device__ __forceinline__ void schur_reg3_body(const TilePlan& tp, const unsigned* __restrict__ p_nit, const int* __restrict__ p_code_start,
                                                const int* __restrict__ p_chunk_start, const unsigned* __restrict__ p_codes, const int* __restrict__ p_obs,
// ... 1128 lines not shown
  const int r = tid >> 4, cl = tid & 15, row = rj + r;
  double a0 = 0.0, a1 = 0.0;
  if (row < n) {
    const double* Tr = Tinv + (long)row * ldw;
    for (int c = rj + cl; c < k0; c += 32) { a0 = fma(Tr[c], Wn[c], a0); a1 = fma(Tr[c + 16], Wn[c + 16], a1); }
  }
  if constexpr (!EARLY) {
    chol_rank_nb(Wn + (k0 - NB), 1, W + (long)k0 * ldw + (k0 - NB), nbp, ldw, sh_red, wv, lane);
    __syncthreads();
  }
#pragma unroll
  for (int h = 0; h < EPT; ++h) {
    const int i = i0 + h * ISTEP;
    if constexpr (EARLY) sh_U[i][j] = m_ij[h];
    else sh_U[i][j] = m_ij[h] - sh_red[(i >> 4) * 2 + (j >> 4)][i & 15][j & 15];
    sh_L[i][j] = l_ij[h];
  }
  __syncthreads();
  if (wv < 2) {
    const int tj = wv;
    v4f64 c = {0.0, 0.0, 0.0, 0.0};
#pragma unroll
    for (int t = 0; t < NB / 4; ++t) {
      const int q = 4 * t + (lane >> 4);
      c = __builtin_amdgcn_mfma_f64_16x16x4f64(sh_U[lane & 15][q], sh_L[tj * 16 + (lane & 15)][q], c, 0, 0, 0);
    }
    if (lane < 16) sh_y[tj * 16 + lane] = (tj * 16 + lane < nbp) ? c[0] : 0.0;
  }
  __syncthreads();
  if (bj < k) {
    chol_rank_nb(Tinv + (long)rj * ldw + (k0 - NB), rcj, W + (long)k0 * ldw + (k0 - NB), nbp, ldw, sh_red, wv, lane);
    __syncthreads();
#pragma unroll
    for (int h = 0; h < EPT; ++h) {
      const int i = i0 + h * ISTEP;
      sh_U[i][j] = (i < rcj && j < nbp) ? old[h] + sh_red[(i >> 4) * 2 + (j >> 4)][i & 15][j & 15] : 0.0;
    }
    __syncthreads();
    if (wv < 4) {
      const int ti = wv >> 1, tj = wv & 1;
      v4f64 c = {0.0, 0.0, 0.0, 0.0};
#pragma unroll
      for (int t = 0; t < NB / 4; ++t) {
        const int q = 4 * t + (lane >> 4);
        c = __builtin_amdgcn_mfma_f64_16x16x4f64(sh_U[ti * 16 + (lane & 15)][q], sh_L[tj * 16 + (lane & 15)][q], c, 0, 0, 0);
      }
#pragma unroll
      for (int rr = 0; rr < 4; ++rr) sh_T[ti * 16 + (lane >> 4) + 4 * rr][tj * 16 + (lane & 15)] = -c[rr];
    }
  } else {
#pragma unroll
    for (int h = 0; h < EPT; ++h) sh_T[i0 + h * ISTEP][j] = old[h];
  }
  __syncthreads();
  if (row < n) {
    const int c = k0 + cl;
    if (c + 16 < n) { a0 = fma(sh_T[r][cl], sh_y[cl], a0); a1 = fma(sh_T[r][cl + 16], sh_y[cl + 16], a1); }
    else if (c < n) a0 = fma(sh_T[r][cl], sh_y[cl], a0);
  }
  double s = a0 + a1;
#pragma unroll
  for (int off = 8; off >= 1; off >>= 1) s += __shfl_xor(s, off, 16);
  if (cl == 0 && row < n) out[row] = s;
}

template <int NC, bool CAMG = false, bool SCAL = false>
__global__ void __launch_bounds__(BLOCK)
k_backsub(const double* __restrict__ obs_u, const double* __restrict__ obs_v, const int* __restrict__ obs_cam,
          const int* __restrict__ obs_pt, const int* __restrict__ pt_start, const int* __restrict__ chunk_start,
          const int* __restrict__ chunk_pts, int n_chunks, const double* __restrict__ xvec, VecLayout lay,
          const double* __restrict__ tab, const int* __restrict__ cam_off, int n_cams, int loss, double f_scale, double lam,
          const double* __restrict__ lam_dev, const double* __restrict__ Vblk, const double* __restrict__ gvec,
          const double* __restrict__ sinv, double* __restrict__ svec, double* __restrict__ step_partial = nullptr) {
  CBA_STAMP(ST_BACKSUB);
  extern __shared__ __attribute__((aligned(16))) double sh[];
  if (lam_dev) lam = *lam_dev;
  double* sh_tab = sh;
  double* sh_dc = sh_tab + (CAMG ? 0 : n_cams * CAMTAB_LDS);
  double* sh_pt = sh_dc + lay.ncp_pad;
  if (!CAMG) stage_camtab(sh_tab, tab, n_cams);
  for (int i = threadIdx.x; i < lay.ncp_pad; i += BLOCK) sh_dc[i] = svec[i];
  __syncthreads();
  for (int c = threadIdx.x; c < n_cams; c += BLOCK) {
    const double* row = tab + (long)c * CAMTAB_DOUBLES;
    double* d3 = sh_dc + (int)row[35];
    const double r0 = d3[0], r1 = d3[1], r2 = d3[2];
    d3[0] = row[12] * r0 + row[13] * r1 + row[14] * r2;
    d3[1] = row[15] * r0 + row[16] * r1 + row[17] * r2;
    d3[2] = row[18] * r0 + row[19] * r1 + row[20] * r2;
  }
  __syncthreads();
  const double* px = xvec + lay.ncp_pad;
  const double* gp = gvec + lay.ncp_pad;
  const double* dp = sinv + lay.ncp_pad;
  double* sp = svec + lay.ncp_pad;
  double sc0 = 0.0, sc1 = 0.0;
  auto solve_point = [&](int p, double* q, const double* Vin, const double* din, const double* gin) {
    double Vd[6], L[6], y[3], x[3];
#pragma unroll
    for (int k = 0; k < 6; ++k) Vd[k] = Vin[k];
    Vd[0] += lam * din[0] * din[0]; Vd[3] += lam * din[1] * din[1]; Vd[5] += lam * din[2] * din[2];
    if (chol3(Vd, L)) {
      chol3_fwd(L, q, y);
      chol3_bwd(L, y, x);
    } else {
      x[0] = x[1] = x[2] = 0.0;
    }
    sp[p] = -x[0];
    sp[lay.Ppad + p] = -x[1];
    sp[2 * lay.Ppad + p] = -x[2];
    if (SCAL) {
#pragma unroll
      for (int k = 0; k < 3; ++k) { const double ps = x[k] * din[k]; sc0 = fma(ps, ps, sc0); sc1 = fma(-gin[k], x[k], sc1); }
    }
  };
  const int last_obs = max(chunk_start[n_chunks] - 1, 0);
  int ch = blockIdx.x;
  int o0 = 0, o1 = 0;
  ObsRec cur = {0.0, 0.0, 0, 0};
  int pt_next = 0;
  double X = 0.0, Yw = 0.0, Zw = 0.0;
  if (ch < n_chunks) {
    o0 = chunk_start[ch]; o1 = chunk_start[ch + 1];
    cur = load_obs(obs_u, obs_v, obs_cam, obs_pt, min(o0 + (int)threadIdx.x, last_obs));
    pt_next = obs_pt[min(chunk_start[min(ch + (int)gridDim.x, n_chunks - 1)] + (int)threadIdx.x, last_obs)];
    X = px[cur.pt]; Yw = px[lay.Ppad + cur.pt]; Zw = px[2 * lay.Ppad + cur.pt];
  }
  while (ch < n_chunks) {
    const int nxt = ch + gridDim.x, nc = min(nxt, n_chunks - 1);
    const int no0 = chunk_start[nc], no1 = chunk_start[nc + 1];
    ObsRec nx;
    {
      const int k1 = min(no0 + (int)threadIdx.x, last_obs);
      nx.u = obs_u[k1]; nx.v = obs_v[k1]; nx.cam = obs_cam[k1]; nx.pt = pt_next;
    }
    const double Xn = px[pt_next], Yn = px[lay.Ppad + pt_next], Zn = px[2 * lay.Ppad + pt_next];
    const int pt_nn = obs_pt[min(chunk_start[min(nxt + (int)gridDim.x, n_chunks - 1)] + (int)threadIdx.x, last_obs)];
    const int cp0 = chunk_pts[2 * ch], npts = chunk_pts[2 * ch + 1];
    const int i = o0 + threadIdx.x;
    const int pp = min(cp0 + (int)threadIdx.x, lay.P - 1);
    int pa = 0, pb = 0;
    double Vp[6] = {0.0, 0.0, 0.0, 0.0, 0.0, 0.0}, dpp[3] = {0.0, 0.0, 0.0}, q[3] = {0.0, 0.0, 0.0}, gq[3] = {0.0, 0.0, 0.0};
    if (threadIdx.x < WAVE) {
      pa = pt_start[pp] - o0; pb = pt_start[pp + 1] - o0;
#pragma unroll
      for (int k = 0; k < 6; ++k) Vp[k] = Vblk[(long)k * lay.Ppad + pp];
#pragma unroll
      for (int k = 0; k < 3; ++k) { dpp[k] = dp[(long)k * lay.Ppad + pp]; q[k] = gp[(long)k * lay.Ppad + pp]; gq[k] = q[k]; }
    }
    double t[3] = {0.0, 0.0, 0.0};
    if (i < o1) {
      const int cam = cur.cam;
      double e[2], G[2][3], Yr[3], Aint[2][3], B[2][3];
      const CamTab& ctb = cam_of<CAMG>(sh_tab, tab, cam);
      obs_factors(ctb, X, Yw, Zw, cur.u, cur.v, loss, f_scale, e, G, Yr, Aint, B);
      const double* dc = sh_dc + (int)ctb.pad[0];
      const double m0 = fma(dc[1], Yr[2], fma(-dc[2], Yr[1], dc[3]));
      const double m1 = fma(dc[2], Yr[0], fma(-dc[0], Yr[2], dc[4]));
      const double m2 = fma(dc[0], Yr[1], fma(-dc[1], Yr[0], dc[5]));
      double a0 = fma(G[0][2], m2, fma(G[0][1], m1, G[0][0] * m0)), a1 = fma(G[1][2], m2, fma(G[1][1], m1, G[1][0] * m0));
      if (NC == 9 && ctb.nparams == 9.0) {
        a0 = fma(Aint[0][2], dc[8], fma(Aint[0][1], dc[7], fma(Aint[0][0], dc[6], a0)));
        a1 = fma(Aint[1][2], dc[8], fma(Aint[1][1], dc[7], fma(Aint[1][0], dc[6], a1)));
      }
      t[0] = B[0][0] * a0 + B[1][0] * a1;
      t[1] = B[0][1] * a0 + B[1][1] * a1;
      t[2] = B[0][2] * a0 + B[1][2] * a1;
    }
    sh_pt[threadIdx.x] = t[0];
    sh_pt[CHUNK + threadIdx.x] = t[1];
    sh_pt[2 * CHUNK + threadIdx.x] = t[2];
    __syncthreads();
    if (npts < 0 && threadIdx.x < 3) {
      double acc = 0.0;
      for (int j = 0; j < o1 - o0; ++j) acc += sh_pt[threadIdx.x * CHUNK + j];
      unsafeAtomicAdd(&sp[(long)threadIdx.x * lay.Ppad + cp0], acc);
    }
    if (threadIdx.x < WAVE && (int)threadIdx.x < npts && pb > pa) {
      for (int j = pa; j < pb; ++j) { q[0] += sh_pt[j]; q[1] += sh_pt[CHUNK + j]; q[2] += sh_pt[2 * CHUNK + j]; }
      solve_point(pp, q, Vp, dpp, gq);
    }
    for (int lp = (threadIdx.x < WAVE ? threadIdx.x + BLOCK : threadIdx.x); lp < npts; lp += BLOCK) {
      const int p = cp0 + lp;
      const int a = pt_start[p] - o0, b = pt_start[p + 1] - o0;
      if (b > a) {
        double q2[3] = {gp[p], gp[lay.Ppad + p], gp[2 * lay.Ppad + p]}, V2[6], d2[3];
        const double g2[3] = {q2[0], q2[1], q2[2]};
        for (int j = a; j < b; ++j) { q2[0] += sh_pt[j]; q2[1] += sh_pt[CHUNK + j]; q2[2] += sh_pt[2 * CHUNK + j]; }
#pragma unroll
        for (int k = 0; k < 6; ++k) V2[k] = Vblk[(long)k * lay.Ppad + p];
#pragma unroll
        for (int k = 0; k < 3; ++k) d2[k] = dp[(long)k * lay.Ppad + p];
        solve_point(p, q2, V2, d2, g2);
      }
    }
    __syncthreads();
    cur = nx; o0 = no0; o1 = no1; ch = nxt;
    pt_next = pt_nn; X = Xn; Yw = Yn; Zw = Zn;
  }
  if (SCAL) {
    double r;
    r = block_sum(sc0, sh_pt); if (threadIdx.x == 0) step_partial[blockIdx.x * 4 + 0] = r;
    r = block_sum(sc1, sh_pt); if (threadIdx.x == 0) { step_partial[blockIdx.x * 4 + 1] = r; step_partial[blockIdx.x * 4 + 2] = 0.0; step_partial[blockIdx.x * 4 + 3] = 0.0; }
  }
}

constexpr int BSR_PT = 3 * CHUNK;
template <int NC> struct BsrCfg {
  static constexpr int NP = SchurRec<NC>::NPH;
  static constexpr int CS = (NC == 9) ? 9 : 8;
  static constexpr int CSS = CS;
  static constexpr size_t lds_bytes(int n_cams) { return ((size_t)BLOCK * NP * 2 + 2 * BSR_PT + (size_t)n_cams * CSS + 8) * sizeof(double); }
};
template <int NC, bool SCAL>
__device__ __forceinline__ void backsub_rec_body(const double* __restrict__ Trec, const int* __restrict__ obs_cam, const int* __restrict__ pt_start,
                                                 const int* __restrict__ chunk_start, const int* __restrict__ chunk_pts, int n_chunks, VecLayout lay,
                                                 const double* __restrict__ tab, const int* __restrict__ cam_off, const int* __restrict__ cam_np,
                                                 int n_cams, double lam, const double* __restrict__ Vblk, const double* __restrict__ gp,
                                                 const double* __restrict__ dp, const double* __restrict__ s_cam, double* __restrict__ sp,
                                                 double* __restrict__ step_partial, double* sh) {
  using Cfg = BsrCfg<NC>;
  constexpr int NP = Cfg::NP, CSS = Cfg::CSS;
  double2* sh_rec = reinterpret_cast<double2*>(sh);
  double* sh_pt = sh + (size_t)BLOCK * NP * 2;
  double* sh_step = sh_pt + 2 * BSR_PT;
  const int tid = (int)threadIdx.x, lane = tid % WAVE;
  const int wv = __builtin_amdgcn_readfirstlane(tid / WAVE);
  for (int idx = tid; idx < n_cams * 3; idx += BLOCK) {
    const int c = idx / 3, a = idx % 3, off = cam_off[c];
    const double* Jl = tab + (long)c * CAMTAB_DOUBLES + 12;
    sh_step[c * CSS + a] = fma(Jl[3 * a + 2], s_cam[off + 2], fma(Jl[3 * a + 1], s_cam[off + 1], Jl[3 * a] * s_cam[off]));
    sh_step[c * CSS + 3 + a] = s_cam[off + 3 + a];
    if (NC == 9) sh_step[c * CSS + 6 + a] = (cam_np[c] == 9) ? s_cam[off + 6 + a] : 0.0;
    if (NC == 6 && a < 2) sh_step[c * CSS + 6 + a] = tab[(long)c * CAMTAB_DOUBLES + 9 + a];
  }
  const int n_obs = chunk_start[n_chunks];
  const int last_obs = max(n_obs - 1, 0);
  const long last_piece = (long)max(n_obs, 1) * NP - 1;
  const double2* rec_g = reinterpret_cast<const double2*>(Trec);
  double2* wrec = sh_rec + wv * (WAVE * NP);
  auto issue = [&](int o0) {
    const long base = ((long)o0 + wv * WAVE) * NP + lane;
#pragma unroll
    for (int k = 0; k < NP; ++k)
      __builtin_amdgcn_global_load_lds((const void __attribute__((address_space(1)))*)(rec_g + min(base + k * WAVE, last_piece)),
                                       (void __attribute__((address_space(3)))*)(wrec + k * WAVE), 16, 0, 0);
  };
  struct PtIn { int p, a, b, on; double V[6], d[3], g[3]; };
  const int lp0 = lane * 4 + wv;
  auto load_point = [&](int cp0, int npts) {
    PtIn q;
    q.on = lp0 < npts;
    q.p = min(cp0 + min(lp0, max(npts - 1, 0)), lay.P - 1);
    q.a = pt_start[q.p]; q.b = pt_start[q.p + 1];
#pragma unroll
    for (int k = 0; k < 6; ++k) q.V[k] = Vblk[(long)k * lay.Ppad + q.p];
#pragma unroll
    for (int k = 0; k < 3; ++k) { q.d[k] = dp[(long)k * lay.Ppad + q.p]; q.g[k] = gp[(long)k * lay.Ppad + q.p]; }
    return q;
  };
  double sc0 = 0.0, sc1 = 0.0;
  auto solve_point = [&](int p, const double* Vin, const double* din, const double* gin, const double* q) {
    double Vd[6], L[6], y[3], x[3];
#pragma unroll
    for (int k = 0; k < 6; ++k) Vd[k] = Vin[k];
    Vd[0] = fma(lam * din[0], din[0], Vd[0]); Vd[3] = fma(lam * din[1], din[1], Vd[3]); Vd[5] = fma(lam * din[2], din[2], Vd[5]);
    if (chol3(Vd, L)) {
      chol3_fwd(L, gin, y);
      y[0] += q[0]; y[1] += q[1]; y[2] += q[2];
      chol3_bwd(L, y, x);
    } else {
      x[0] = x[1] = x[2] = 0.0;
    }
    sp[p] = -x[0];
    sp[lay.Ppad + p] = -x[1];
    sp[2 * lay.Ppad + p] = -x[2];
    if (SCAL) {
#pragma unroll
      for (int k = 0; k < 3; ++k) { const double ps = x[k] * din[k]; sc0 = fma(ps, ps, sc0); sc1 = fma(-gin[k], x[k], sc1); }
    }
  };
  auto point_phase = [&](const PtIn& q, const double* pt, int cp0, int npts, int o0) {
    if (q.on && q.b > q.a) {
      double acc[3] = {0.0, 0.0, 0.0};
      for (int j = q.a - o0; j < q.b - o0; ++j) { acc[0] += pt[j]; acc[1] += pt[CHUNK + j]; acc[2] += pt[2 * CHUNK + j]; }
      solve_point(q.p, q.V, q.d, q.g, acc);
    }
    for (int lp = tid + BLOCK; lp < npts; lp += BLOCK) {
      const int p = cp0 + lp, a = pt_start[p] - o0, b = pt_start[p + 1] - o0;
      if (b > a) {
        double acc[3] = {0.0, 0.0, 0.0}, V2[6], d2[3], g2[3];
        for (int j = a; j < b; ++j) { acc[0] += pt[j]; acc[1] += pt[CHUNK + j]; acc[2] += pt[2 * CHUNK + j]; }
#pragma unroll
        for (int k = 0; k < 6; ++k) V2[k] = Vblk[(long)k * lay.Ppad + p];
#pragma unroll
        for (int k = 0; k < 3; ++k) { d2[k] = dp[(long)k * lay.Ppad + p]; g2[k] = gp[(long)k * lay.Ppad + p]; }
        solve_point(p, V2, d2, g2, acc);
      }
    }
  };

  int ch = blockIdx.x;
  if (ch >= n_chunks) {
    if (SCAL && tid == 0) { step_partial[blockIdx.x * 4 + 0] = 0.0; step_partial[blockIdx.x * 4 + 1] = 0.0; step_partial[blockIdx.x * 4 + 2] = 0.0; step_partial[blockIdx.x * 4 + 3] = 0.0; }
    return;
  }
  struct Ent { int o0, o1, cp0, npts; };
  auto load_ent = [&](int c) { Ent e; e.o0 = chunk_start[c]; e.o1 = chunk_start[c + 1]; e.cp0 = chunk_pts[2 * c]; e.npts = chunk_pts[2 * c + 1]; return e; };
  const int stride = (int)gridDim.x, last_chunk = n_chunks - 1;
// ... 1316 lines not shown
```

### caliscope_amd/csrc/cba_lib.hip

```cpp
#include <hip/hip_runtime.h>

#include <algorithm>
#include <atomic>
#include <chrono>
#include <cmath>
#include <condition_variable>
#include <cstdarg>
#include <cstdio>
#include <cstdlib>
#include <cstring>
#include <map>
#include <mutex>
#include <shared_mutex>
#include <memory>
#include <string>
#include <type_traits>
#include <thread>
#include <utility>
#include <vector>

#include <rccl/rccl.h>
#include <rocprofiler-sdk-roctx/roctx.h>

#include "../../include/caliscope_ba.h"
// ... 561 lines not shown
  std::sort(rows.begin(), rows.end(), [](const Row& a, const Row& b) { return a.t0 < b.t0; });
  size_t first = 0;
  for (size_t i = 0; i < rows.size(); ++i) if (rows[i].slot == ST_TPREP) first = i;
  fprintf(stderr, "device stamps of the last fused iteration (100 MHz wall clock; blocks = workgroups seen, at most %d):\n", STAMP_BLOCKS);
  fprintf(stderr, "| # | kernel | workgroups | first entry -> last exit, us | last entry after the first, us | workgroup lifetime min / mean / max, us | idle before, us |\n|---|---|---|---|---|---|---|\n");
  double busy = 0.0, idle = 0.0;
  for (size_t i = first; i < rows.size(); ++i) {
    const Row& r = rows[i];
    char nm[48];
    if (r.slot == ST_CHOL_STEP + 1 && chol_pairs(p)) snprintf(nm, sizeof nm, "k_chol_step k=-1 and 0");
    else if (r.slot >= ST_CHOL_STEP) snprintf(nm, sizeof nm, "k_chol_step k=%d", r.slot - ST_CHOL_STEP - 1); else snprintf(nm, sizeof nm, "%s", names[r.slot]);
    const double gap = i > first ? (r.t0 - rows[i - 1].t1) * 0.01 : 0.0;
    busy += (r.t1 - r.t0) * 0.01; if (i > first) idle += gap;
    fprintf(stderr, "| %zu | %s | %d | %.2f | %.2f | %.2f / %.2f / %.2f | %.2f |\n", i - first + 1, nm, r.blocks, (r.t1 - r.t0) * 0.01, (r.last_entry - r.t0) * 0.01,
            r.life_min * 0.01, r.life_sum / r.blocks * 0.01, r.life_max * 0.01, gap);
  }
  for (size_t i = 0; i < first; ++i) {
    const Row& r = rows[i];
    if (r.slot != ST_JV) continue;
    fprintf(stderr, "| (earlier) | %s | %d | %.2f | %.2f | %.2f / %.2f / %.2f | - |\n", names[r.slot], r.blocks, (r.t1 - r.t0) * 0.01,
            (r.last_entry - r.t0) * 0.01, r.life_min * 0.01, r.life_sum / r.blocks * 0.01, r.life_max * 0.01);
  }
  if (first < rows.size())
    fprintf(stderr, "%zu kernels, %.1f us inside kernels, %.1f us between them, %.1f us from the first entry to the last exit\n", rows.size() - first, busy, idle,
            (rows.back().t1 - rows[first].t0) * 0.01);
  if (!p->h_tile_wg_begin.empty() && p->tile_grid <= STAMP_BLOCKS) {
    const std::vector<int>& wgb = p->h_tile_wg_begin;
    const int nT = (int)wgb.size() - 1;
    std::vector<double> life(p->tile_grid, 0.0);
    for (int b = 0; b < p->tile_grid; ++b) {
      const long long* q = &h[((size_t)ST_PAIRS * STAMP_BLOCKS + b) * STAMP_ROW];
      long long e = 0;
      for (int w = 0; w < STAMP_WAVES; ++w) e = std::max(e, q[1 + w]);
      life[logical_workgroup(b, p->tile_grid)] = q[0] ? (e - q[0]) * 0.01 : 0.0;
    }
    fprintf(stderr, "k_schur_reg3 workgroup lifetimes by tile (us): tile: workgroups min / mean / max\n");
    for (int t = 0; t < nT; ++t) {
      double mn = 1e300, mx = 0.0, sm = 0.0;
      for (int b = wgb[t]; b < wgb[t + 1]; ++b) { mn = std::min(mn, life[b]); mx = std::max(mx, life[b]); sm += life[b]; }
      fprintf(stderr, "  %d: %d  %.1f / %.1f / %.1f\n", t, wgb[t + 1] - wgb[t], mn, sm / std::max(1, wgb[t + 1] - wgb[t]), mx);
    }
    fprintf(stderr, "... by XCD (logical id mod 8): min / mean / max\n");
    for (int x = 0; x < 8; ++x) {
      double mn = 1e300, mx = 0.0, sm = 0.0; int n = 0;
      for (int b = x; b < p->tile_grid; b += 8) { mn = std::min(mn, life[b]); mx = std::max(mx, life[b]); sm += life[b]; ++n; }
      fprintf(stderr, "  XCD %d: %.1f / %.1f / %.1f\n", x, mn, sm / std::max(1, n), mx);
    }
    fprintf(stderr, "... by dispatch order (hardware workgroup id, eighths of the grid): mean\n ");
    for (int o = 0; o < 8; ++o) {
      double sm = 0.0; int n = 0;
      for (int b = o * p->tile_grid / 8; b < (o + 1) * p->tile_grid / 8; ++b) { sm += life[logical_workgroup(b, p->tile_grid)]; ++n; }
      fprintf(stderr, " %.1f", sm / std::max(1, n));
    }
    fprintf(stderr, "\n");
  }
  (void)hipFree(p->stamps);
  p->stamps = nullptr;
}
#endif

void cba_destroy(cba_problem* p) {
  if (!p) return;
  drop_plan_task(p);
  (void)hipSetDevice(p->device);
  if (p->stream) (void)hipStreamSynchronize(p->stream);
  upload_stage_release(p);
#ifdef CBA_PROFILING
  if (p->stamps) dump_stamps(p);
#endif
  drain_timers(p);
  for (auto& ev : p->free_events) { (void)hipEventDestroy(ev.a); (void)hipEventDestroy(ev.b); }
  if (p->h_vec_sent) (void)hipEventDestroy(p->h_vec_sent);
  if (ncclComm_t c = p->comm.exchange(nullptr)) (void)ncclCommDestroy(c);
  {
    std::lock_guard<std::mutex> lock(g_pool_mu);
    DevicePool& pool = g_pool[p->device];
    for (size_t i = 0; i < p->allocs.size(); ++i) {
      if (p->alloc_bytes[i] == kPoolChunk && pool.chunks.size() < kPoolKeep) pool.chunks.push_back(p->allocs[i]);
      else (void)hipFree(p->allocs[i]);
    }
    if (p->h_scal) {
      if (pool.mail.size() < kPoolKeep) pool.mail.emplace_back(p->h_scal, p->mail_doubles);
      else (void)hipHostFree(p->h_scal);
    }
    if (p->h_vec) {
      if (pool.staging.size() < kPoolKeep && p->h_vec_doubles <= kPoolStagingMax) pool.staging.emplace_back(p->h_vec, p->h_vec_doubles);
      else (void)hipHostFree(p->h_vec);
    }
    if (p->stream) {
      if (pool.streams.size() < kPoolKeep) pool.streams.push_back(p->stream);
      else (void)hipStreamDestroy(p->stream);
    }
  }
  delete p;
}

}

static int raise_lds_ceiling(const void* fn, size_t bytes) {
  static std::mutex mu;
  static std::map<std::pair<int, const void*>, size_t> ceiling;
  int dev = 0;
  HIPCHK(hipGetDevice(&dev));
  std::lock_guard<std::mutex> lock(mu);
  size_t& have = ceiling[{dev, fn}];
  if (bytes <= have) return CBA_OK;
  HIPCHK(hipFuncSetAttribute(fn, hipFuncAttributeMaxDynamicSharedMemorySize, (int)bytes));
  have = bytes;
  return CBA_OK;
}

template <int NC> constexpr bool LIN_FORM = NC == 6;
template <int NC> static bool linear_pass_now(const cba_problem* p) { return LIN_FORM<NC> && p->linear_pass && p->loss == LOSS_LINEAR; }

template <typename K>
static int allow_lds(K kernel, size_t bytes) {
  if (bytes > 160 * 1024) return fail(CBA_ERR_UNSUPPORTED, "kernel needs %zu bytes of LDS (> 160 KiB)", bytes);
  return raise_lds_ceiling(reinterpret_cast<const void*>(kernel), bytes);
}

template <typename K>
static int resident_per_cu(K kernel, size_t lds, int fallback) {
  int n = 0;
  if (hipOccupancyMaxActiveBlocksPerMultiprocessor(&n, kernel, BLOCK, lds) != hipSuccess || n <= 0) { (void)hipGetLastError(); return fallback; }
  return std::min(n, 8);
}

static size_t lds_tab(const cba_problem* p) { return p->tab_global ? 0 : (size_t)p->C * CAMTAB_LDS; }
static size_t lds_cost(const cba_problem* p) { return (lds_tab(p) + 8) * 8; }
template <int NC> static size_t lds_build_camg(const cba_problem* p) { return ((size_t)p->C * UPack<NC>::STRIDE + 9 * CHUNK + 8) * 8; }
template <int NC> static bool build_camg(const cba_problem* p) {
  if (p->tab_global) return true;
  const size_t with_tab = ((size_t)p->C * CAMTAB_LDS + (size_t)p->C * UPack<NC>::STRIDE + 9 * CHUNK + 8) * 8;
  if (const char* e = std::getenv("CBA_BUILD_CAMG")) return std::atoi(e) != 0 && !p->det_m;
  return !p->det_m && ((with_tab > 80 * 1024 && lds_build_camg<NC>(p) <= 80 * 1024) || with_tab > 160 * 1024);
}
template <int NC> static size_t lds_build_cs(const cba_problem* p, bool camg, bool uglob = false) {
  return ((camg ? 0 : (size_t)p->C * CAMTAB_LDS) + (uglob ? 0 : (size_t)p->C * UPack<NC>::STRIDE) + 12 * (size_t)p->cs.pmax + 8) * 8;
}
template <int NC> static bool build_cs_uglob(const cba_problem* p) { return lds_build_cs<NC>(p, true) > 160 * 1024; }
template <int NC> static bool build_cs_camg(const cba_problem* p) { return p->tab_global || lds_build_cs<NC>(p, false) > 80 * 1024; }
template <int NC> static size_t lds_build(const cba_problem* p) {
  if (build_camg<NC>(p)) return lds_build_camg<NC>(p);
  if (p->det_m)
    return ((size_t)p->C * CAMTAB_LDS + (size_t)DET_ROUND * DET_LD + 9 * CHUNK + 8) * 8 + ((size_t)CHUNK + p->C + 1) * 4;
  return ((size_t)p->C * CAMTAB_LDS + (size_t)p->C * UPack<NC>::STRIDE + 9 * CHUNK + 8) * 8;
}
static size_t lds_jv(const cba_problem* p, int nv) { return (lds_tab(p) + (size_t)nv * p->lay.ncp_pad + 8) * 8; }
template <int NC> struct RegCfg;
template <> struct RegCfg<6> { static constexpr int SPLIT = 1, MINW = 2, PER_CU = 2; };
template <> struct RegCfg<9> { static constexpr int SPLIT = 3, MINW = 3, PER_CU = 1; };
template <int NC> static size_t lds_tprep(const cba_problem* p) {
  if (p->det_m) return ((size_t)SchurRec<NC>::STAGE_WAVES * WAVE * SchurRec<NC>::STAGE * 2 + (size_t)p->C * CAMTAB_LDS + (size_t)DET_ROUND * DET_LD) * 8 + ((size_t)CHUNK + p->C + 1) * 4;
  return ((size_t)SchurRec<NC>::STAGE_WAVES * WAVE * SchurRec<NC>::STAGE * 2 + lds_tab(p) + p->lay.ncp_pad) * 8;
}
constexpr int kSchurRegMaxGroup = 16;
constexpr size_t kSmallSolveLds = ((size_t)(SMALL_N + 1) * SMALL_LD + (size_t)2 * NB * (NB + 1) + (size_t)((SMALL_N + NB - 1) / NB) * NB * (NB + 1) + 2 * SMALL_N) * 8;
static size_t lds_backsub(const cba_problem* p) { return (lds_tab(p) + p->lay.ncp_pad + 3 * CHUNK) * 8; }
template <int NC> static size_t lds_backsub_rec(const cba_problem* p) { return BsrCfg<NC>::lds_bytes(p->C); }


static bool plan_timing_on() {
  static const bool on = std::getenv("CBA_PLAN_TIMING") != nullptr;
  return on;
}

template <int NC, typename KCfg>
static Reg2Params reg2_params(const cba_problem* p) {
  Reg2Params prm;
  const int g = p->gsz;
  prm.C = p->C; prm.P = p->P; prm.G = p->G; prm.g = g;
  constexpr int CT = KCfg::CODE_THREADS;
  prm.rep = (g * g <= CT / 2) ? CT / (g * g) : 1;
  prm.n_waves = KCfg::CODE_WAVES;
  prm.pair_cap = KCfg::PAIR_CAP;
  prm.chunk_cap = KCfg::SCHUNK;
  prm.slots_per_wave = KCfg::EPW; prm.wave_pieces = KCfg::WAVE_PIECES; prm.rec_pieces = KCfg::LST;
  prm.zero_piece = KCfg::ZERO_PIECE;
  prm.heavy_obs = p->n_heavy ? HEAVY_OBS : 0;
  if (const char* e = std::getenv("CBA_PLAN_REGION")) prm.region_chunks = std::max(1, std::min(std::atoi(e), 1024));
  return prm;
}

struct PlanInstall {
  TilePlan tp{};
  int tile_grid = 0, n_tile_chunks = 0, reg_reduce_y = 4;
  long tile_stream_len = 0, n_pairs = 0;
  double lane_util = 0.0;
  int* tile_wg_begin = nullptr;
  std::vector<int> h_wgb;
  std::vector<std::pair<void*, size_t>> owned;
  int rc = CBA_OK;
};

template <int NC, typename KCfg, typename Upload>
static int prepare_install(const cba_problem* p, Reg2Plan& plan, const Reg2Params& prm, int max_blocks, Upload&& upload, PlanInstall& out) {
  const int G = p->G, g = p->gsz, C = p->C;
  const int nT = p->n_tiles;
  const bool plan_timing = plan_timing_on();
  auto t_now = []() { return std::chrono::duration<double>(std::chrono::steady_clock::now().time_since_epoch()).count(); };
  double t_mark = t_now();
  auto lap = [&](const char* what) { if (plan_timing) { const double t = t_now(); fprintf(stderr, "  plan: %-34s %.3f s\n", what, t - t_mark); t_mark = t; } };
  constexpr int CT = KCfg::CODE_THREADS;
  out.n_tile_chunks = plan.tile_chunk_begin[nT];
  out.tile_stream_len = (long)plan.obs.size() - 2 * KCfg::SCHUNK;
  out.n_pairs = plan.n_pairs;
  out.lane_util = plan.lane_iters > 0 ? (double)plan.n_pairs / (double)plan.lane_iters : 0.0;
  if (plan_timing)
    fprintf(stderr, "  plan: %d tiles x %d regions, %d chunks (%.1f slots each), %ld pairs, lane utilisation %.3f, LDS cycles per 16-lane read group %.2f (arrival order %.2f)\n",
            nT, plan.n_regions, out.n_tile_chunks, out.n_tile_chunks ? (double)out.tile_stream_len / out.n_tile_chunks : 0.0, plan.n_pairs, out.lane_util,
            plan.lds_groups ? (double)plan.lds_cycles / plan.lds_groups : 0.0, plan.lds_groups ? (double)plan.lds_cycles_arrival / plan.lds_groups : 0.0);
  const double cost_a = 2.0;
  std::vector<float> chunk_cost;
  const std::vector<double> tile_cost = cba::tile_costs(plan.nit, plan.tile_chunk_begin, nT, KCfg::CODE_WAVES, KCfg::REG_BLOCK / KCfg::SPLIT / WAVE, cost_a, &chunk_cost);
  const char* bind_env = std::getenv("CBA_BIND");
  const WgBinding bind = cba::bind_workgroups(plan.tile_chunk_begin, nT, max_blocks, true, &tile_cost, &chunk_cost, bind_env && bind_env[0] == 'f');
  out.tile_grid = bind.grid;
  lap("workgroup binding");
  std::vector<int> gcam(G + 1), gpar(G + 1), ta(nT), tb(nT);
  for (int a = 0; a <= G; ++a) {
    gcam[a] = std::min(a * g, C);
    gpar[a] = (gcam[a] < C) ? p->h_cam_off[gcam[a]] : p->ncp;
  }
  {
    int t = 0;
    for (int a = 0; a < G; ++a)
      for (int b = a; b < G; ++b, ++t) { ta[t] = a; tb[t] = b; }
  }
  int rc;
  int *dob = nullptr, *dcs = nullptr, *dcode = nullptr, *dwf = nullptr, *dwt = nullptr, *dwe = nullptr, *dws = nullptr, *dta = nullptr, *dtb = nullptr,
      *dgc = nullptr, *dgp = nullptr;
  unsigned *dcodes = nullptr, *dnit = nullptr;
#define TRYP(e) do { rc = (e); if (rc) return rc; } while (0)
  TRYP(upload(&dob, plan.obs)); TRYP(upload(&dcs, plan.chunk_start)); TRYP(upload(&dcode, plan.code_start));
  TRYP(upload(&dcodes, plan.codes)); TRYP(upload(&dnit, plan.nit));
  TRYP(upload(&dwf, bind.wfirst)); TRYP(upload(&dwt, bind.wt)); TRYP(upload(&dwe, bind.wend)); TRYP(upload(&dws, bind.wstride));
  TRYP(upload(&dta, ta)); TRYP(upload(&dtb, tb)); TRYP(upload(&dgc, gcam)); TRYP(upload(&dgp, gpar));
  TRYP(upload(&out.tile_wg_begin, bind.wgb));
#undef TRYP
  out.h_wgb = bind.wgb;
  {
    int rows = 0;
    for (int t = 0; t < nT; ++t) rows = std::max(rows, (bind.wgb[t + 1] - bind.wgb[t]) * std::max(prm.rep, 1));
    out.reg_reduce_y = rows > 96 ? REG_REDUCE_Y_MAX : 4;
  }
  lap("upload");
  TilePlan tp{};
  tp.chunk_start = dcs; tp.wg_first = dwf; tp.wg_end = dwe; tp.wg_tile = dwt; tp.wg_stride = dws; tp.tile_a = dta; tp.tile_b = dtb;
  tp.group_cam_begin = dgc; tp.group_par_begin = dgp; tp.g = g;
  tp.tile_elems = CT * p->nct * p->nct; tp.obs = dob; tp.rep = prm.rep;
  tp.codes = dcodes; tp.code_start = dcode; tp.nit = dnit;
  tp.prio_shift = (NC == 6) ? 0 : -1;
  if (const char* e = std::getenv("CBA_PAIR_PRIO")) tp.prio_shift = std::atoi(e);
  out.tp = tp;
  return CBA_OK;
}

static void apply_install(cba_problem* p, PlanInstall& in) {
  p->tp = in.tp;
  p->tile_grid = in.tile_grid; p->n_tile_chunks = in.n_tile_chunks; p->reg_reduce_y = in.reg_reduce_y;
  p->tile_stream_len = in.tile_stream_len; p->n_pairs = in.n_pairs; p->plan_lane_util = in.lane_util;
  p->tile_wg_begin = in.tile_wg_begin;
  p->h_tile_wg_begin = std::move(in.h_wgb);
  for (auto& o : in.owned) { p->allocs.push_back(o.first); p->alloc_bytes.push_back(o.second); p->device_bytes += (long)o.second; }
  in.owned.clear();
}

static int prepare_install_background(const cba_problem* p, Reg2Plan& plan, const Reg2Params& prm, PlanInstall& in) {
  if (hipSetDevice(p->device) != hipSuccess) return CBA_ERR_HIP;
  auto upload = [&](auto** out, const auto& h) -> int {
    using T = typename std::remove_pointer<typename std::remove_pointer<decltype(out)>::type>::type;
    const size_t bytes = std::max<size_t>(h.size(), 1) * sizeof(T);
    void* ptr = nullptr;
    if (hipMalloc(&ptr, bytes) != hipSuccess) return CBA_ERR_HIP;
    in.owned.emplace_back(ptr, bytes);
    if (!h.empty() && hipMemcpy(ptr, h.data(), h.size() * sizeof(T), hipMemcpyHostToDevice) != hipSuccess) return CBA_ERR_HIP;
    *out = static_cast<T*>(ptr);
    return CBA_OK;
  };
  return (p->nct == 9) ? prepare_install<9, Reg3Cfg<9>>(p, plan, prm, p->plan_max_blocks, upload, in)
                       : prepare_install<6, Reg3Cfg<6>>(p, plan, prm, p->plan_max_blocks, upload, in);
}

struct PlanTask {
  Reg2Params prm;
  Reg2Plan cheap, plan;
  PlanInstall install;
  const cba_problem* handle = nullptr;
  int rc_cheap = 0, rc = 0;
  double seconds_cheap = 0.0, seconds = 0.0;
  bool two_stage = false;
  std::atomic<int> stage{0};
  std::atomic<bool> cancel{false};
  std::mutex mu;
  std::condition_variable cv;
  std::thread th;
  HostVec<int> hcam_keep;
  std::vector<int> hps_keep;
  void start(const Reg2Params& params, const int* hcam, const int* hps, bool two, const cba_problem* h) {
    prm = params;
    handle = h;
    prm.cancel = &cancel;
    two_stage = two;
    th = std::thread([this, hcam, hps] {
      auto publish = [this](int s) { { std::lock_guard<std::mutex> lock(mu); stage.store(s, std::memory_order_release); } cv.notify_all(); };
      if (two_stage) {
        const auto t0 = std::chrono::steady_clock::now();
// ... 1928 lines not shown
```

Measured before the change: 4.140 billion obs/s.

## Reorder LDS camera rows into aligned 16-byte pieces and load only needed fields

Moves the camera table into a new LDS row layout of 38 doubles: 16-byte aligned, an odd number of 2-double pieces, and fields reordered so each kernel reads a prefix of pieces with 128-bit LDS loads. Camera data is copied into registers once per observation rather than read through references. The per-camera RHS accumulator in tprep also gets its own padded, bank-friendly stride, with the J_l transform and scatter done per task at the end. The aim is to cut LDS bank conflicts and load count in the hot per-observation kernels, at the cost of more complex index mapping and slightly more LDS per camera.

```diff
diff --git a/caliscope_amd/build.py b/caliscope_amd/build.py
--- a/caliscope_amd/build.py
+++ b/caliscope_amd/build.py
@@ -11,7 +11,7 @@
 CSRC = HERE / "csrc"
 OUT = HERE / "libcaliscope_ba.so"
 SOURCES = [CSRC / "cba_lib.hip", CSRC / "cba_solve.cpp", CSRC / "pose_lib.hip", CSRC / "scale_lib.hip", CSRC / "coverage_lib.hip", CSRC / "vertical_lib.hip", CSRC / "report_lib.hip", CSRC / "trajectory_lib.hip", CSRC / "covariance_lib.hip", CSRC / "reliability_lib.hip"]
-DEPENDS = [CSRC / "cba_kernels.h", CSRC / "schur_plan.h", CSRC / "chol_schedule.h", CSRC / "chol_factor.h", CSRC / "host_plan.h", CSRC / "wg_binding.h", CSRC / "ba_math.h", CSRC / "trf_math.h", CSRC / "pnp_math.h", CSRC / "epipolar_math.h", CSRC / "intrinsic_math.h", CSRC / "frame_select_math.h", CSRC / "scale_math.h", CSRC / "coverage_math.h", CSRC / "vertical_math.h", CSRC / "report_math.h", CSRC / "trajectory_math.h", CSRC / "trajectory_refine_math.h", CSRC / "trajectory_cov_math.h", CSRC / "trajectory_smooth_math.h", CSRC / "covariance_math.h", CSRC / "covariance_constraint_math.h", CSRC / "covariance_constraint_plan.h", CSRC / "covariance_pipeline.h", CSRC / "reliability_math.h", CSRC / "reliability_constraint_math.h", CSRC / "device_call.h",
+DEPENDS = [CSRC / "cba_kernels.h", CSRC / "schur_plan.h", CSRC / "chol_schedule.h", CSRC / "chol_factor.h", CSRC / "host_plan.h", CSRC / "wg_binding.h", CSRC / "ba_math.h", CSRC / "camera_row.h", CSRC / "trf_math.h", CSRC / "pnp_math.h", CSRC / "epipolar_math.h", CSRC / "intrinsic_math.h", CSRC / "frame_select_math.h", CSRC / "scale_math.h", CSRC / "coverage_math.h", CSRC / "vertical_math.h", CSRC / "report_math.h", CSRC / "trajectory_math.h", CSRC / "trajectory_refine_math.h", CSRC / "trajectory_cov_math.h", CSRC / "trajectory_smooth_math.h", CSRC / "covariance_math.h", CSRC / "covariance_constraint_math.h", CSRC / "covariance_constraint_plan.h", CSRC / "covariance_pipeline.h", CSRC / "reliability_math.h", CSRC / "reliability_constraint_math.h", CSRC / "device_call.h",
            HERE.parent / "include" / "caliscope_ba.h", HERE.parent / "include" / "caliscope_pose.h", HERE.parent / "include" / "caliscope_coverage.h", HERE.parent / "include" / "caliscope_vertical.h", HERE.parent / "include" / "caliscope_report.h", HERE.parent / "include" / "caliscope_trajectory.h", HERE.parent / "include" / "caliscope" / "uncertainty.h", HERE.parent / "include" / "caliscope" / "uncertainty_constrained.h",HERE.parent / "include" / "caliscope" / "reliability.h", HERE.parent / "include" / "caliscope" / "reliability_constrained.h",HERE.parent / "include" / "caliscope" / "trajectory_refine.h", HERE.parent / "include" / "caliscope" / "trajectory_uncertainty.h", HERE.parent / "include" / "caliscope" / "trajectory_smoother.h"]
 ARCH = "gfx950"
 
diff --git a/caliscope_amd/csrc/ba_math.h b/caliscope_amd/csrc/ba_math.h
--- a/caliscope_amd/csrc/ba_math.h
+++ b/caliscope_amd/csrc/ba_math.h
@@ -130,7 +130,8 @@
   L->xr2 = L->yr2 = L->xr4 = L->yr4 = 0.0;
 }
 
-CBA_HD void project_residual(const CamTab& c, double X, double Y, double Z, double u, double v, double* e) {
+template <typename Cam>
+CBA_HD void project_residual(const Cam& c, double X, double Y, double Z, double u, double v, double* e) {
   const double Xc = c.t[0] + c.R[0] * X + c.R[1] * Y + c.R[2] * Z;
   const double Yc = c.t[1] + c.R[3] * X + c.R[4] * Y + c.R[5] * Z;
   const double Zc = c.t[2] + c.R[6] * X + c.R[7] * Y + c.R[8] * Z;
diff --git a/caliscope_amd/csrc/camera_row.h b/caliscope_amd/csrc/camera_row.h
--- /dev/null
+++ b/caliscope_amd/csrc/camera_row.h
@@ -0,0 +1,69 @@
+#pragma once
+#include "ba_math.h"
+
+namespace cba {
+
+constexpr int CAMTAB_LIVE = 36;
+constexpr int CAMTAB_LDS = 38;
+constexpr int CAMROW_PIECES = CAMTAB_LDS / 2;
+static_assert(CAMTAB_LDS % 2 == 0 && CAMROW_PIECES % 2 == 1, "rows start on 16 bytes; an odd number of pieces per row");
+
+constexpr int CAMROW_R = 0, CAMROW_T = 9, CAMROW_FX = 12, CAMROW_FY = 13, CAMROW_D = 14, CAMROW_INV_FX0 = 19, CAMROW_MODEL = 20, CAMROW_NPARAMS = 21,
+              CAMROW_OFF = 22, CAMROW_CX = 23, CAMROW_CY = 24, CAMROW_FX0 = 25, CAMROW_FY0 = 26, CAMROW_JL = 28;
+constexpr int CAMROW_PIECES_LIN6 = 12;
+constexpr int CAMROW_PIECES_RES6 = 13;
+constexpr int CAMROW_PIECES_FULL = 14;
+constexpr int CAMROW_JL_PIECE = CAMROW_JL / 2, CAMROW_JL_PIECES = 5;
+static_assert(CAMROW_JL % 2 == 0 && CAMROW_JL_PIECE + CAMROW_JL_PIECES == CAMROW_PIECES, "J_l is a run of whole pieces at the end of the row");
+
+CBA_HD constexpr int camrow_index(int i) {
+  return i < 12 ? i
+       : i < 21 ? CAMROW_JL + (i - 12)
+       : i < 23 ? CAMROW_FX + (i - 21)
+       : i < 25 ? CAMROW_CX + (i - 23)
+       : i < 30 ? CAMROW_D + (i - 25)
+       : i < 32 ? CAMROW_FX0 + (i - 30)
+       : CAMROW_INV_FX0 + (i - 32);
+}
+CBA_HD constexpr int camrow_source(int j) {
+  return j < 12 ? j
+       : j < 14 ? 21 + (j - CAMROW_FX)
+       : j < 19 ? 25 + (j - CAMROW_D)
+       : j < 23 ? 32 + (j - CAMROW_INV_FX0)
+       : j < 25 ? 23 + (j - CAMROW_CX)
+       : j < 27 ? 30 + (j - CAMROW_FX0)
+       : j < 28 ? -1
+       : j < 37 ? 12 + (j - CAMROW_JL)
+       : -1;
+}
+
+struct alignas(16) CamRowLds {
+  double R[9], t[3];
+  double fx, fy;
+  double d[5];
+  double inv_fx0, model, nparams, off;
+  double cx, cy, fx0, fy0, unused0;
+  double Jl[9], unused1;
+};
+static_assert(sizeof(CamRowLds) == CAMTAB_LDS * sizeof(double), "CamRowLds is one LDS row");
+static_assert(offsetof(CamRowLds, t) == CAMROW_T * 8 && offsetof(CamRowLds, fx) == CAMROW_FX * 8 && offsetof(CamRowLds, d) == CAMROW_D * 8 &&
+                  offsetof(CamRowLds, inv_fx0) == CAMROW_INV_FX0 * 8 && offsetof(CamRowLds, model) == CAMROW_MODEL * 8 &&
+                  offsetof(CamRowLds, nparams) == CAMROW_NPARAMS * 8 && offsetof(CamRowLds, off) == CAMROW_OFF * 8 &&
+                  offsetof(CamRowLds, cx) == CAMROW_CX * 8 && offsetof(CamRowLds, fx0) == CAMROW_FX0 * 8 && offsetof(CamRowLds, Jl) == CAMROW_JL * 8,
+              "CamRowLds follows the CAMROW_ indices");
+
+CBA_HD void camrow_pack(const double* tab_row, double* lds_row) {
+  for (int j = 0; j < CAMTAB_LDS; ++j) lds_row[j] = camrow_source(j) >= 0 ? tab_row[camrow_source(j)] : 0.0;
+}
+CBA_HD void camrow_put_piece(CamTab* c, int k, double lo, double hi) {
+  double* dst = reinterpret_cast<double*>(c);
+  if (camrow_source(2 * k) >= 0) dst[camrow_source(2 * k)] = lo;
+  if (camrow_source(2 * k + 1) >= 0) dst[camrow_source(2 * k + 1)] = hi;
+}
+
+CBA_HD constexpr int camacc_stride(int nc) { return nc | 1; }
+CBA_HD constexpr int camacc_index(int nc, int cam, int r) { return cam * camacc_stride(nc) + r; }
+CBA_HD constexpr int camacc_tasks(int nc, int n_cams) { return n_cams * camacc_stride(nc); }
+CBA_HD void camacc_task(int nc, int task, int* cam, int* r) { *cam = task / camacc_stride(nc); *r = task % camacc_stride(nc); }
+
+}
diff --git a/caliscope_amd/csrc/cba_kernels.h b/caliscope_amd/csrc/cba_kernels.h
--- a/caliscope_amd/csrc/cba_kernels.h
+++ b/caliscope_amd/csrc/cba_kernels.h
@@ -2,6 +2,7 @@
 #include <hip/hip_runtime.h>
 
 #include "ba_math.h"
+#include "camera_row.h"
 #include "trf_math.h"
 #include "wg_binding.h"
 #include "chol_schedule.h"
@@ -80,8 +81,6 @@
 
 __device__ __forceinline__ void lds_add(double* addr, double v) { unsafeAtomicAdd(addr, v); }
 
-constexpr int CAMTAB_LIVE = 36;
-constexpr int CAMTAB_LDS = CAMTAB_LIVE + 1;
 struct ObsRec { double u, v; int cam, pt; };
 __device__ __forceinline__ ObsRec load_obs(const double* __restrict__ obs_u, const double* __restrict__ obs_v,
                                            const int* __restrict__ obs_cam, const int* __restrict__ obs_pt, int i) {
@@ -91,17 +90,69 @@
 }
 
 __device__ __forceinline__ void stage_camtab(double* sh_tab, const double* tab, int n_cams) {
-  for (int i = threadIdx.x; i < n_cams * CAMTAB_LIVE; i += BLOCK)
-    sh_tab[(i / CAMTAB_LIVE) * CAMTAB_LDS + (i % CAMTAB_LIVE)] = tab[(i / CAMTAB_LIVE) * CAMTAB_DOUBLES + (i % CAMTAB_LIVE)];
-}
-__device__ __forceinline__ const CamTab& cam_at(const double* sh_tab, int cam) {
-  return *reinterpret_cast<const CamTab*>(sh_tab + cam * CAMTAB_LDS);
-}
+  for (int i = threadIdx.x; i < n_cams * CAMTAB_LDS; i += BLOCK) {
+    const int c = i / CAMTAB_LDS, src = camrow_source(i % CAMTAB_LDS);
+    sh_tab[i] = src >= 0 ? tab[c * CAMTAB_DOUBLES + src] : 0.0;
+  }
+}
+enum CamRead : int { CAM_READ_PIECES = 0, CAM_READ_ALIGNED = 1 };
+typedef double cam_piece_t __attribute__((ext_vector_type(2)));
 template <bool CAMG>
-__device__ __forceinline__ const CamTab& cam_of(const double* sh_tab, const double* __restrict__ tab, int cam) {
-  if constexpr (CAMG) return *reinterpret_cast<const CamTab*>(tab + (long)cam * CAMTAB_DOUBLES);
-  else return cam_at(sh_tab, cam);
-}
+struct CamRef {
+  const double* row;
+  template <int NPIECES, bool JL = false, CamRead HOW = CAM_READ_PIECES>
+  __device__ __forceinline__ CamTab load() const {
+    CamTab c;
+    double* dst = reinterpret_cast<double*>(&c);
+#pragma unroll
+    for (int i = 0; i < CAMTAB_DOUBLES; ++i) dst[i] = 0.0;
+    if constexpr (CAMG) {
+#pragma unroll
+      for (int i = 0; i < 12; ++i) dst[i] = row[i];
+      if constexpr (JL) {
+#pragma unroll
+        for (int i = 12; i < 21; ++i) dst[i] = row[i];
+      }
+      dst[21] = row[21]; dst[22] = row[22];
+      if constexpr (NPIECES > CAMROW_PIECES_LIN6) { dst[23] = row[23]; dst[24] = row[24]; }
+#pragma unroll
+      for (int i = 25; i < 35; ++i) dst[i] = row[i];
+    } else if constexpr (HOW != CAM_READ_PIECES) {
+      const double* src = static_cast<const double*>(__builtin_assume_aligned(row, 16));
+#pragma unroll
+      for (int j = 0; j < CAMTAB_LDS; ++j)
+        if ((j < 2 * NPIECES || (JL && j >= CAMROW_JL)) && camrow_source(j) >= 0) dst[camrow_source(j)] = src[j];
+    } else {
+      const cam_piece_t* P = reinterpret_cast<const cam_piece_t*>(row);
+#pragma unroll
+      for (int k = 0; k < CAMROW_PIECES; ++k) {
+        if (k < NPIECES || (JL && k >= CAMROW_JL_PIECE)) {
+          const cam_piece_t p = P[k];
+          camrow_put_piece(&c, k, p.x, p.y);
+        }
+      }
+    }
+    return c;
+  }
+  __device__ __forceinline__ int off(const CamTab& c) const { return (int)(CAMG ? row[35] : c.pad[0]); }
+  __device__ __forceinline__ void jl(double* J) const {
+    if constexpr (CAMG) {
+#pragma unroll
+      for (int i = 0; i < 9; ++i) J[i] = row[12 + i];
+    } else {
+      const cam_piece_t* P = reinterpret_cast<const cam_piece_t*>(row) + CAMROW_JL_PIECE;
+      const cam_piece_t a = P[0], b = P[1], c = P[2], d = P[3], e = P[4];
+      J[0] = a.x; J[1] = a.y; J[2] = b.x; J[3] = b.y; J[4] = c.x; J[5] = c.y; J[6] = d.x; J[7] = d.y; J[8] = e.x;
+    }
+  }
+  __device__ __forceinline__ double nparams() const { return row[CAMG ? 34 : CAMROW_NPARAMS]; }
+};
+template <bool CAMG>
+__device__ __forceinline__ CamRef<CAMG> cam_of(const double* sh_tab, const double* __restrict__ tab, int cam) {
+  if constexpr (CAMG) return CamRef<true>{tab + (long)cam * CAMTAB_DOUBLES};
+  else return CamRef<false>{sh_tab + cam * CAMTAB_LDS};
+}
+template <int NC, bool LIN = false> constexpr int CAM_PIECES = NC == 6 ? (LIN ? CAMROW_PIECES_LIN6 : CAMROW_PIECES_RES6) : CAMROW_PIECES_FULL;
 
 __global__ void k_cam_prep(const double* __restrict__ xvec, const double* __restrict__ cam_const,
                            const int* __restrict__ cam_model, const int* __restrict__ cam_np,
@@ -175,7 +226,8 @@
     const Rec rnn = load_rec(i + 2 * stride);
     __builtin_amdgcn_sched_barrier(0);
     double e[2];
-    project_residual(cam_of<CAMG>(sh_tab, tab, rc.cam), X, Y, Z, rc.u, rc.v, e);
+    if constexpr (CAMG) project_residual(*reinterpret_cast<const CamTab*>(tab + (long)rc.cam * CAMTAB_DOUBLES), X, Y, Z, rc.u, rc.v, e);
+    else project_residual(*reinterpret_cast<const CamRowLds*>(sh_tab + rc.cam * CAMTAB_LDS), X, Y, Z, rc.u, rc.v, e);
     if (!(isfinite(e[0]) && isfinite(e[1]))) bad = true;
     acc += robust_cost_one(loss, f_scale, e[0]) + robust_cost_one(loss, f_scale, e[1]);
     if (WRITE_R) {
@@ -314,10 +366,9 @@
 }
 
 template <int NC>
-__device__ __forceinline__ double obs_linearize(const CamTab& c_lds, double X, double Y, double Z, double u, double v,
+__device__ __forceinline__ double obs_linearize(const CamTab& c, double X, double Y, double Z, double u, double v,
                                                 int loss, double f_scale, double* e, double (*A)[MAX_NC],
                                                 double (*B)[3]) {
-  const CamTab c = c_lds;
   __builtin_amdgcn_sched_barrier(0);
   project_full(c, X, Y, Z, u, v, e, A, B);
   double rho = 0.0;
@@ -335,17 +386,8 @@
   return rho;
 }
 
-__device__ __forceinline__ double obs_factors(const CamTab& c_lds, double X, double Y, double Z, double u, double v, int loss, double f_scale, double* e,
+__device__ __forceinline__ double obs_factors(const CamTab& c, double X, double Y, double Z, double u, double v, int loss, double f_scale, double* e,
                                               double (*G)[3], double* Yr, double (*Aint)[3], double (*B)[3], double* nrm = nullptr) {
-  CamTab c;
-  {
-    const double* src = reinterpret_cast<const double*>(&c_lds);
-    double* dst = reinterpret_cast<double*>(&c);
-#pragma unroll
-    for (int i = 0; i < 12; ++i) dst[i] = src[i];
-#pragma unroll
-    for (int i = 21; i < 35; ++i) dst[i] = src[i];
-  }
   __builtin_amdgcn_sched_barrier(0);
   project_factors(c, X, Y, Z, u, v, e, G, Yr, Aint, B, nrm);
   if (nrm) {
@@ -365,18 +407,8 @@
   }
   return rho;
 }
-__device__ __forceinline__ void obs_factors(const CamTab& c_lds, double X, double Y, double Z, double (*G)[3], double* Yr, double (*Aint)[3], double (*B)[3],
+__device__ __forceinline__ void obs_factors(const CamTab& c, double X, double Y, double Z, double (*G)[3], double* Yr, double (*Aint)[3], double (*B)[3],
                                             double* nrm = nullptr) {
-  CamTab c;
-  {
-    const double* src = reinterpret_cast<const double*>(&c_lds);
-    double* dst = reinterpret_cast<double*>(&c);
-#pragma unroll
-    for (int i = 0; i < 12; ++i) dst[i] = src[i];
-    dst[21] = src[21]; dst[22] = src[22];
-#pragma unroll
-    for (int i = 25; i < 35; ++i) dst[i] = src[i];
-  }
   __builtin_amdgcn_sched_barrier(0);
   project_factors(c, X, Y, Z, G, Yr, Aint, B, nrm);
 #pragma unroll
@@ -451,9 +483,6 @@
   extern __shared__ __attribute__((aligned(16))) double sh[];
   double* sh_tab = sh;
   double* sh_U = sh_tab + (CAMG ? 0 : n_cams * CAMTAB_LDS);
-  auto cam_of = [&](int cam) -> const CamTab& {
-    return CAMG ? *reinterpret_cast<const CamTab*>(tab + (long)cam * CAMTAB_DOUBLES) : cam_at(sh_tab, cam);
-  };
   double* sh_pt = sh_U + (DET ? DET_ROUND * DET_LD : n_cams * UP::STRIDE);
   double* sh_red = sh_pt + 9 * CHUNK;
   int* sh_perm = reinterpret_cast<int*>(sh_red + 8);
@@ -503,7 +532,8 @@
     if (i < o1) {
       const int cam = cur.cam, pt = cur.pt;
       double B[2][3];
-      cost += obs_linearize<NC>(cam_of(cam), px[pt], px[lay.Ppad + pt], px[2 * lay.Ppad + pt], cur.u, cur.v, loss,
+      const CamTab ctl = cam_of<CAMG>(sh_tab, tab, cam).template load<CAM_PIECES<NC>, true>();
+      cost += obs_linearize<NC>(ctl, px[pt], px[lay.Ppad + pt], px[2 * lay.Ppad + pt], cur.u, cur.v, loss,
                                 f_scale, e, A, B);
       if (!isfinite(e[0] + e[1])) bad = true;
       pv[0] = B[0][0] * B[0][0] + B[1][0] * B[1][0];
@@ -515,7 +545,7 @@
       pv[6] = B[0][0] * e[0] + B[1][0] * e[1];
       pv[7] = B[0][1] * e[0] + B[1][1] * e[1];
       pv[8] = B[0][2] * e[0] + B[1][2] * e[1];
-      const int np = (int)cam_of(cam).nparams;
+      const int np = (int)ctl.nparams;
       np_det = np;
       if (!DET) {
         double* Uc = sh_U + cam * UP::STRIDE;
@@ -685,19 +715,23 @@
       const double u = n_u, v = n_v;
       n_cam = cs.cam[min(j + 1, jl)]; n_pl = cs.ptl[min(j + 1, jl)]; n_u = cs.u[min(j + 1, jl)]; n_v = cs.v[min(j + 1, jl)];
       __builtin_amdgcn_sched_barrier(0);
-      if (cam != cur_cam) { flush(); cur_cam = cam; cur_np = (int)cam_of<CAMG>(sh_tab, tab, cam).nparams; }
+      const CamRef<CAMG> rfc = cam_of<CAMG>(sh_tab, tab, cam);
+      if constexpr (CAMG) { if (cam != cur_cam) { flush(); cur_cam = cam; cur_np = (int)rfc.nparams(); } }
       double e[2], A[2][MAX_NC], B[2][3];
       {
         double G[2][3], Yr[3], Aint[2][3];
-        const CamTab& ctc = cam_of<CAMG>(sh_tab, tab, cam);
+        const CamTab ctc = rfc.template load<CAM_PIECES<NC>>();
+        if constexpr (!CAMG) { if (cam != cur_cam) { flush(); cur_cam = cam; cur_np = (int)ctc.nparams; } }
         cost += obs_factors(ctc, sh_x[pl], sh_x[PM + pl], sh_x[2 * PM + pl], u, v, loss, f_scale, e, G, Yr, Aint, B);
 #pragma unroll
         for (int r = 0; r < 2; ++r) {
           const double p0 = Yr[1] * G[r][2] - Yr[2] * G[r][1], p1 = Yr[2] * G[r][0] - Yr[0] * G[r][2], p2 = Yr[0] * G[r][1] - Yr[1] * G[r][0];
           if constexpr (UGLOB) {
-            A[r][0] = ctc.Jl[0] * p0 + ctc.Jl[3] * p1 + ctc.Jl[6] * p2;
-            A[r][1] = ctc.Jl[1] * p0 + ctc.Jl[4] * p1 + ctc.Jl[7] * p2;
-            A[r][2] = ctc.Jl[2] * p0 + ctc.Jl[5] * p1 + ctc.Jl[8] * p2;
+            double Jl[9];
+            rfc.jl(Jl);
+            A[r][0] = Jl[0] * p0 + Jl[3] * p1 + Jl[6] * p2;
+            A[r][1] = Jl[1] * p0 + Jl[4] * p1 + Jl[7] * p2;
+            A[r][2] = Jl[2] * p0 + Jl[5] * p1 + Jl[8] * p2;
           } else {
             A[r][0] = p0; A[r][1] = p1; A[r][2] = p2;
           }
@@ -964,10 +998,11 @@
     __builtin_amdgcn_sched_barrier(0);
     const int cam = rc.cam;
     double e[2], G[2][3], Yr[3], Aint[2][3], B[2][3];
-    const CamTab& ctj = cam_of<CAMG>(sh_tab, tab, cam);
+    const CamRef<CAMG> rfj = cam_of<CAMG>(sh_tab, tab, cam);
+    const CamTab ctj = rfj.template load<CAM_PIECES<NC, LIN>>();
     if constexpr (LIN) obs_factors(ctj, gc.X, gc.Y, gc.Z, G, Yr, Aint, B);
     else obs_factors(ctj, gc.X, gc.Y, gc.Z, rc.u, rc.v, loss, f_scale, e, G, Yr, Aint, B);
-    const double* vc = sh_v + (int)ctj.pad[0];
+    const double* vc = sh_v + rfj.off(ctj);
     auto jv = [&](const double* q, double px0, double px1, double px2, double* o0, double* o1) {
       const double m0 = fma(q[1], Yr[2], fma(-q[2], Yr[1], q[3]));
       const double m1 = fma(q[2], Yr[0], fma(-q[0], Yr[2], q[4]));
@@ -981,12 +1016,20 @@
       }
       *o0 = a0; *o1 = a1;
     };
+    auto jv6 = [&](const double* q, double px0, double px1, double px2, double* o0, double* o1) {
+      if constexpr (NC == 6 && NV == 1 && !CAMG) {
+        const cam_piece_t* Q = reinterpret_cast<const cam_piece_t*>(q);
+        const cam_piece_t q0 = Q[0], q1 = Q[1], q2 = Q[2];
+        const double w[6] = {q0.x, q0.y, q1.x, q1.y, q2.x, q2.y};
+        jv(w, px0, px1, px2, o0, o1);
+      } else jv(q, px0, px1, px2, o0, o1);
+    };
     double a0, a1;
-    jv(vc, gc.a, gc.b, gc.c, &a0, &a1);
+    jv6(vc, gc.a, gc.b, gc.c, &a0, &a1);
     s11 += a0 * a0 + a1 * a1;
     if (NV == 2) {
       double b0, b1;
-      jv(vc + lay.ncp_pad, gc.d, gc.e, gc.f, &b0, &b1);
+      jv6(vc + lay.ncp_pad, gc.d, gc.e, gc.f, &b0, &b1);
       s12 += a0 * b0 + a1 * b1;
       s22 += b0 * b0 + b1 * b1;
     }
@@ -1134,9 +1177,9 @@
   double dacc[DM];
 #pragma unroll
   for (int m = 0; m < DM; ++m) dacc[m] = 0.0;
-  stage_camtab(sh_tab, tab, n_cams);
+  if (!CAMG) stage_camtab(sh_tab, tab, n_cams);
   if (!DET)
-    for (int i = threadIdx.x; i < lay.ncp_pad; i += BLOCK) sh_b[i] = 0.0;
+    for (int i = threadIdx.x; i < camacc_tasks(NC, n_cams); i += BLOCK) sh_b[i] = 0.0;
   __syncthreads();
   const double* px = xvec + lay.ncp_pad;
   const double* gp = gvec + lay.ncp_pad;
@@ -1227,7 +1270,8 @@
     }
     if (i < o1) {
       const int cam = cur.cam;
-      const CamTab& ct = cam_of<CAMG>(sh_tab, tab, cam);
+      const CamRef<CAMG> rft = cam_of<CAMG>(sh_tab, tab, cam);
+      const CamTab ct = rft.template load<(NC == 6 && LIN) ? CAMROW_PIECES_LIN6 - 1 : CAM_PIECES<NC, LIN>, false, CAM_READ_ALIGNED>();
       const double X = ops.X, Yw = ops.Y, Zw = ops.Z;
       double e[2], G[2][3], Yr[3], Aint[2][3], B[2][3], Z[2][3], nrm[3];
       if constexpr (LIN) obs_factors(ct, X, Yw, Zw, G, Yr, Aint, B, NC == 6 ? nrm : nullptr);
@@ -1247,7 +1291,7 @@
       const double gpt[3] = {ops.g[0], ops.g[1], ops.g[2]};
       double y[3];
       chol3_fwd(L, gpt, y);
-      double* bc = sh_b + (int)ct.pad[0];
+      double* bc = sh_b + camacc_index(NC, cam, 0);
       rec[0] = Yr[0]; rec[1] = Yr[1]; rec[2] = Yr[2];
       double qy[3];
       if constexpr (NC == 6) {
@@ -1285,8 +1329,10 @@
       {
         const double c0 = Yr[1] * qy[2] - Yr[2] * qy[1], c1 = Yr[2] * qy[0] - Yr[0] * qy[2], c2 = Yr[0] * qy[1] - Yr[1] * qy[0];
         if (DET) {
-#pragma unroll
-          for (int r = 0; r < 3; ++r) bval[r] = ct.Jl[r] * c0 + ct.Jl[3 + r] * c1 + ct.Jl[6 + r] * c2;
+          double Jl[9];
+          rft.jl(Jl);
+#pragma unroll
+          for (int r = 0; r < 3; ++r) bval[r] = Jl[r] * c0 + Jl[3 + r] * c1 + Jl[6 + r] * c2;
         } else {
           lds_add(&bc[0], c0); lds_add(&bc[1], c1); lds_add(&bc[2], c2);
         }
@@ -1338,18 +1384,18 @@
     for (int m = 0; m < DM; ++m) {
       const int task = (int)threadIdx.x + BLOCK * m;
       const int c = task / DET_ROUND, q = task % DET_ROUND;
-      if (task < n_cams * DET_ROUND && q < (int)cam_at(sh_tab, c).nparams) brow[cam_off[c] + q] = dacc[m];
+      if (task < n_cams * DET_ROUND && q < (int)sh_tab[c * CAMTAB_LDS + CAMROW_NPARAMS]) brow[cam_off[c] + q] = dacc[m];
     }
   } else {
-    for (int c = threadIdx.x; c < n_cams; c += BLOCK) {
+    for (int i = lay.ncp + threadIdx.x; i < lay.ncp_pad; i += BLOCK) brow[i] = 0.0;
+    for (int task = threadIdx.x; task < camacc_tasks(NC, n_cams); task += BLOCK) {
+      int c, r;
+      camacc_task(NC, task, &c, &r);
       const double* row = tab + (long)c * CAMTAB_DOUBLES;
-      double* b3 = sh_b + (int)row[35];
-      const double c0 = b3[0], c1 = b3[1], c2 = b3[2];
-#pragma unroll
-      for (int r = 0; r < 3; ++r) b3[r] = row[12 + r] * c0 + row[15 + r] * c1 + row[18 + r] * c2;
-    }
-    __syncthreads();
-    for (int i = threadIdx.x; i < lay.ncp_pad; i += BLOCK) brow[i] = sh_b[i];
+      if (r >= (int)row[34]) continue;
+      const double* b3 = sh_b + camacc_index(NC, c, 0);
+      brow[(int)row[35] + r] = r < 3 ? row[12 + r] * b3[0] + row[15 + r] * b3[1] + row[18 + r] * b3[2] : b3[r];
+    }
   }
 }
 
@@ -2784,9 +2830,10 @@
     if (i < o1) {
       const int cam = cur.cam;
       double e[2], G[2][3], Yr[3], Aint[2][3], B[2][3];
-      const CamTab& ctb = cam_of<CAMG>(sh_tab, tab, cam);
+      const CamRef<CAMG> rfb = cam_of<CAMG>(sh_tab, tab, cam);
+      const CamTab ctb = rfb.template load<CAM_PIECES<NC>>();
       obs_factors(ctb, X, Yw, Zw, cur.u, cur.v, loss, f_scale, e, G, Yr, Aint, B);
-      const double* dc = sh_dc + (int)ctb.pad[0];
+      const double* dc = sh_dc + rfb.off(ctb);
       const double m0 = fma(dc[1], Yr[2], fma(-dc[2], Yr[1], dc[3]));
       const double m1 = fma(dc[2], Yr[0], fma(-dc[0], Yr[2], dc[4]));
       const double m2 = fma(dc[0], Yr[1], fma(-dc[1], Yr[0], dc[5]));
diff --git a/caliscope_amd/csrc/cba_lib.hip b/caliscope_amd/csrc/cba_lib.hip
--- a/caliscope_amd/csrc/cba_lib.hip
+++ b/caliscope_amd/csrc/cba_lib.hip
@@ -737,7 +737,7 @@
 template <> struct RegCfg<9> { static constexpr int SPLIT = 3, MINW = 3, PER_CU = 1; };
 template <int NC> static size_t lds_tprep(const cba_problem* p) {
   if (p->det_m) return ((size_t)SchurRec<NC>::STAGE_WAVES * WAVE * SchurRec<NC>::STAGE * 2 + (size_t)p->C * CAMTAB_LDS + (size_t)DET_ROUND * DET_LD) * 8 + ((size_t)CHUNK + p->C + 1) * 4;
-  return ((size_t)SchurRec<NC>::STAGE_WAVES * WAVE * SchurRec<NC>::STAGE * 2 + lds_tab(p) + p->lay.ncp_pad) * 8;
+  return ((size_t)SchurRec<NC>::STAGE_WAVES * WAVE * SchurRec<NC>::STAGE * 2 + lds_tab(p) + (size_t)camacc_tasks(NC, p->C)) * 8;
 }
 constexpr int kSchurRegMaxGroup = 16;
 constexpr size_t kSmallSolveLds = ((size_t)(SMALL_N + 1) * SMALL_LD + (size_t)2 * NB * (NB + 1) + (size_t)((SMALL_N + NB - 1) / NB) * NB * (NB + 1) + 2 * SMALL_N) * 8;
```

New measurement: 4.195 billion obs/s (median of 6 runs). +1.3%, better.
